# haowenz/FEM

Hardware: AMD Instinct MI355X
Metric: mapped Mreads/s (100 bp, e=3) at 1/2/4/8 MI355X + achieved HBM GB/s vs roofline (higher is better)
Workload: dtype u32/u64 integer + 32-bit Myers bit-vectors

## Files before the change

### fem_amd/csrc/fem_hip.hip

```cpp
#include "../../include/fem_hip.h"

#include <hip/hip_runtime.h>
#include <rccl/rccl.h>
#include <sched.h>
#if defined(__x86_64__)
#include <immintrin.h>
#endif

#include <algorithm>
#include <cctype>
#include <cstdio>
#include <cstdlib>
#include <cstring>
#include <condition_variable>
#include <functional>
#include <memory>
#include <atomic>
#include <chrono>
#include <mutex>
#include <string>
#include <thread>
#include <utility>
#include <vector>

#include "fem_buf.hip.h"
#include "fem_index_build.hip.h"
#include "fem_pack.h"
#include "fem_kernels.hip.h"
#include "fem_verify.hip.h"
#include "fem_seed_fast.hip.h"
#include "fem_seed_join.hip.h"
#include "fem_tail.hip.h"
#include "fem_bgzf.hip.h"

namespace {

using femb::Buf;
using femb::Event;
using femb::PinBuf;
using femb::Stream;
template <typename T>
using StageBuf = femb::Buf<T, femb::Mem::Device, femb::Grow::Half>;
template <typename T>
using PinStageBuf = femb::Buf<T, femb::Mem::Pinned, femb::Grow::Half>;

#ifndef FEM_SLOTS
#define FEM_SLOTS 4
#endif
constexpr int kSlots = FEM_SLOTS;
constexpr uint32_t kMaxReadLen = 1024;
constexpr size_t kFrontPad = 16;
constexpr size_t kPackedFrontPad = 256;
constexpr uint32_t kXcapSmall = 512, kFcap = 128, kCcap = 128;

constexpr int kTimedKernels = 16;
struct TimedLaunch {
  int kernel;
  hipEvent_t start, stop;
  bool counts = true;
};
constexpr int kMaxParts = 4;

struct Slot {
  Stream stream;
  StageBuf<uint8_t> d_bases_alloc;
  uint8_t *bases() const { return d_bases_alloc + 16; }
  StageBuf<uint64_t> d_off;
  uint64_t n_reads = 0;
  uint64_t n_bases = 0;
  uint32_t max_len = 0;
  bool staged = false;
  PinStageBuf<char> h_bases;
  PinStageBuf<uint64_t> h_off;
  uint64_t acq_reads = 0, acq_bases = 0;
  PinStageBuf<char> h_quals, h_names;
  PinStageBuf<uint64_t> h_name_off;
  StageBuf<uint8_t> d_quals, d_names;
  StageBuf<uint64_t> d_name_off;
  bool text_staged = false;
  bool host_quals = false;
  const uint64_t *qual_at = nullptr;
  Stream text_stream;
  Stream out_stream;
  Event ev_text_staged;
  Event ev_text_order;
  bool have_text_order = false;
  StageBuf<uint8_t> d_packed_alloc;
  uint8_t *packed() const { return d_packed_alloc + kPackedFrontPad; }
  StageBuf<uint32_t> d_exc_bits;
  uint32_t packed_bpr = 0;
  bool prefetch_results = false, staged_by_copy = false;
  uint64_t prefetched_reads2 = 0, prefetched_cand = 0, last_n_cand = 0;
  uint64_t h2d_bytes = 0;
  bool sent_packed = false;
  int parts = 1;
  uint32_t part_begin[kMaxParts + 1] = {0, 0, 0, 0, 0};
  Event ev_part[kMaxParts], ev_sel[kMaxParts];
  Event ev_zeroed;
  Event ev_results, ev_home;
  Buf<uint64_t> d_cand;
  Buf<uint32_t> d_meta;
  Buf<uint8_t> d_ed;
  Buf<int16_t> d_end;
  uint32_t cand_cap = 0;
  Buf<uint32_t> d_begin, d_count, d_nmap;
  Buf<uint8_t> d_ctl;
  PinBuf<uint8_t> h_ctl;
  Buf<uint64_t> d_arena;
  uint64_t arena_cap = 0;
  Buf<uint32_t> d_slow;
  uint32_t slow_cap = 0;
  StageBuf<uint2> d_sel, d_sel_hdr;
  PinBuf<uint32_t> h_begin, h_count;
  PinBuf<uint64_t> h_cand;
  PinBuf<uint8_t> h_ed;
  PinBuf<int16_t> h_end;
  StageBuf<uint8_t> d_count8;
  StageBuf<uint32_t> d_seg;
  Buf<uint64_t> d_pcand;
  Buf<uint8_t> d_ped;
  Buf<int16_t> d_pend;
  Buf<uint2> d_big;
  PinBuf<uint8_t> h_count8, h_ped;
  PinBuf<uint32_t> h_seg;
  PinBuf<uint64_t> h_pcand;
  PinBuf<int16_t> h_pend;
  PinBuf<uint2> h_big;
  bool want_packed = false;
  bool packed_enqueued = false;
  uint64_t packed_home = 0, last_n_packed = 0;
  bool packed_per_read_home = false;
  uint32_t n_packed = 0, n_big = 0;
  fem_params params{};
  bool mapped = false, synced = false;
  uint64_t stats[5] = {0, 0, 0, 0, 0};
  uint32_t n_cand = 0;
  std::vector<TimedLaunch> pending;
  std::unique_ptr<femt::Tail> tail;
  bool paired = false;
  int32_t min_insert = 0, max_insert = 0;
  uint64_t n_proper = 0;
  bool rescue = false;
  int32_t rescue_edits = 0;
  uint64_t n_rescued = 0;
  bool mapq = false;
  bool unmapped = false;
  uint64_t n_unmapped = 0;
  int32_t report_strata = -1, report_hits = -1;
  uint64_t n_filtered = 0;
  std::vector<uint16_t> pr_flag;
  std::vector<uint32_t> pr_tid, pr_pos0, pr_cigar_off, pr_cigar, pr_md_off;
  std::vector<uint8_t> pr_nm;
  std::vector<char> pr_md;
};

constexpr size_t kCtlPackCursor = 4 * sizeof(uint32_t) + 2 * sizeof(uint64_t) + 4 * sizeof(uint64_t);
constexpr size_t kCtlBytes = kCtlPackCursor + 2 * sizeof(uint32_t);
constexpr uint32_t kBigCap = 4096;
constexpr size_t kCtlWorkCursor = 128, kCtlWorkCursor2 = 192, kCtlPartStride = 128, kCtlAlloc = 1024;
static_assert(kCtlWorkCursor2 + (kMaxParts - 1) * kCtlPartStride + 64 <= kCtlAlloc, "control block layout");
static_assert(kCtlBytes <= kCtlWorkCursor, "control block layout");

}

namespace {
class StagePool {
 public:
  ~StagePool() {
    {
      std::lock_guard<std::mutex> l(m_);
      stop_ = true;
    }
    cv_.notify_all();
    for (auto &t : threads_) t.join();
  }
  void run(unsigned n, const std::function<void(unsigned)> &work) {
    if (n <= 1) return work(0u);
    {
      std::lock_guard<std::mutex> l(m_);
      while (threads_.size() + 1 < n) {
        const unsigned id = (unsigned)threads_.size() + 1;
        threads_.emplace_back([this, id] { loop(id); });
      }
      work_ = &work, n_ = n, pending_ = n - 1, ++epoch_;
    }
    cv_.notify_all();
    work(0u);
    std::unique_lock<std::mutex> l(m_);
    done_.wait(l, [&] { return pending_ == 0; });
    work_ = nullptr;
  }

 private:
  void loop(unsigned id) {
    uint64_t seen = 0;
    for (;;) {
      const std::function<void(unsigned)> *w = nullptr;
      {
        std::unique_lock<std::mutex> l(m_);
        cv_.wait(l, [&] { return stop_ || (epoch_ != seen && id < n_); });
        if (stop_) return;
        seen = epoch_, w = work_;
      }
      (*w)(id);
      std::lock_guard<std::mutex> l(m_);
      if (--pending_ == 0) done_.notify_one();
    }
  }
  std::mutex m_;
  std::condition_variable cv_, done_;
  std::vector<std::thread> threads_;
  const std::function<void(unsigned)> *work_ = nullptr;
  unsigned n_ = 0, pending_ = 0;
  uint64_t epoch_ = 0;
  bool stop_ = false;
};
}

struct fem_dev {
  femt::TextGate text_gate;
  std::unique_ptr<femz::Bgzf> bgzf;
  Buf<uint8_t> d_zin;
  Stream z_stream;
  std::recursive_mutex mu;
  int device = 0;
  std::unique_ptr<StagePool> stage_pool;
  Buf<uint8_t> d_ref_names;
  Buf<uint32_t> d_ref_name_off;
  int n_cu = 256;
  std::string err;
  Buf<uint32_t> d_lookup;
  uint64_t n_lookup = 0;
  Buf<uint64_t> d_occ;
  uint64_t n_occ = 0;
  int32_t k = 0, step = 0;
  uint64_t fast_occ_key = ~0ull;
  int fast_occ_blocks = 0;
  Buf<uint32_t> d_summary;
  Buf<uint32_t> d_occ32, d_goff, d_blkseq;
  uint32_t list_shift = 0;
  bool no_strided = false;
  bool verify_chars = false;
  Buf<uint32_t> d_freq11;
  uint32_t n_banks = 1, bank_first[5] = {0, 0, 0, 0, 0};
  Buf<uint32_t> d_bank_lo;
  uint64_t bank_limit = 0;
  uint32_t bank_seqs = 0;
  int select_occ_blocks = 0, join_occ_blocks = 0;
  uint64_t select_occ_key = ~0ull, join_occ_key = ~0ull;
  Buf<uint8_t> d_planes;
  Buf<uint8_t> d_ref_raw;
  uint64_t ref_bytes = 0;
  Buf<uint64_t> d_seq_off;
  Buf<uint32_t> d_seq_len;
  uint32_t n_seq = 0;
  std::vector<uint64_t> seq_off;
  std::vector<uint32_t> seq_len;
  Slot slot[kSlots];
  bool timing = false;
  int verify_blocks_per_cu = 0;
  int verify_packed_blocks_per_cu = 0;
  double t_ms[kTimedKernels] = {};
  uint64_t t_n[kTimedKernels] = {};
  bool force_generic = false;
  bool force_hash = false;
  bool force_dense = false;
  bool no_dense = false;
  bool tiny_buffers = false;
  femb::EventPool event_pool;
  Event ev_kernels_done;
  bool have_kernels_done = false;
  Event ev_select_done;
  bool have_select_done = false;
  bool no_overlap = false;
  Event ev_h2d_done;
  bool have_h2d_done = false;
  Stream side_stream;
  bool no_parts = false;
  int max_parts = 2;
  bool timeline = false, have_epoch = false;
  Event ev_epoch;
};

namespace {

bool testing_switch(const char *name) {
  const char *t = getenv("FEM_TESTING");
  if (!(t && t[0] == '1')) return false;
  const char *v = getenv(name);
  return v && v[0] == '1';
}

int fail(fem_dev *h, int rc, const std::string &msg) {
  if (h) {
    std::lock_guard<std::recursive_mutex> lock(h->mu);
    h->err = msg;
  }
  return rc;
}
#define FEM_LOCK(h) std::lock_guard<std::recursive_mutex> fem_lock_(h->mu)

#define HIP_TRY(h, expr)                                                                          \
  do {                                                                                            \
    hipError_t e_ = (expr);                                                                       \
    if (e_ != hipSuccess)                                                                         \
      return fail(h, e_ == hipErrorOutOfMemory ? FEM_ERR_NOMEM : FEM_ERR_HIP,                     \
                  std::string(#expr) + ": " + hipGetErrorString(e_));                             \
  } while (0)

bool params_ok(const fem_params *p) {
  return p && p->k >= 1 && p->k <= 15 && p->step >= 1 && p->step <= 16 && p->e >= 0 && p->e <= 7 && p->a >= 0 &&
         p->a <= 2;
}

femk::SeedLayout make_layout(const fem_params &p, uint32_t max_len) {
  femk::SeedLayout l{};
  const uint32_t R = (uint32_t)(p.e + 1 + p.a);
  const uint32_t lg = (uint32_t)(p.k / p.step + (p.k % p.step ? 1 : 0));
  const uint32_t n_groups = 2u * (uint32_t)p.step;
  uint32_t smax = max_len >= (uint32_t)p.k ? max_len - (uint32_t)p.k + 1u : 1u;
  int c = (int)(smax / (uint32_t)p.step) - (int)(R * lg) + 2;
  uint32_t cmax = (uint32_t)std::max(c, 2);
  l.smax = smax;
  l.cmax = cmax;
  l.cw = (cmax + 31u) / 32u;
  l.n_words = (max_len + 15u) / 16u + 2u;
  l.xcap = kXcapSmall, l.fcap = kFcap, l.ccap = kCcap;
  uint32_t o = 0;
  auto take = [&](uint32_t bytes) {
    uint32_t at = o;
    o += (bytes + 15u) & ~15u;
    return at;
  };
  l.pkw = take(l.n_words * 4u);
  l.nkw = take(l.n_words * 4u);
  l.sf = take(2u * smax * 8u);
  l.dp_rows = take(n_groups * 2u * cmax * 4u);
  l.dp_bits = take(std::max(n_groups * R * l.cw * 4u, n_groups * R * 8u));
  l.picked = take(n_groups * R * 16u);
  l.rb = take(2u * (R + 1u) * 4u);
  l.X = take(l.xcap * 8u);
  l.F = take(l.fcap * 8u);
  l.A = take(l.ccap * 8u);
  l.B = take(l.ccap * 8u);
  l.wave_bytes = o;
  return l;
}

femk::SeedLayout make_layout_fast(const fem_params &p, uint32_t max_len, bool hash) {
  femk::SeedLayout l{};
  const uint32_t R = (uint32_t)(p.e + 1 + p.a);
  const uint32_t n_groups = 2u * (uint32_t)p.step;
  l.smax = max_len >= (uint32_t)p.k ? max_len - (uint32_t)p.k + 1u : 1u;
  l.n_words = (max_len + 15u) / 16u + 2u;
  l.xcap = 64;
  uint32_t o = 0;
  auto take = [&](uint32_t bytes) {
    uint32_t at = o;
    o += (bytes + 15u) & ~15u;
    return at;
  };
  if (hash) {
    l.pkw = take(l.n_words * 4u);
    l.nkw = take(l.n_words * 4u);
  }
  if (hash) l.sf = take(std::max(2u * l.smax * 8u, 2u * 64u * 8u));
  l.dp_bits = take(std::max(n_groups, femk::kGroupQueue) * R * 8u);
  if (hash) {
    l.X = take(64u * 8u);
    l.A = take(femk::kListScratchBytes);
  }
  l.B = take(2u * femk::kReadBlock * 8u);
  if (!hash) {
    const uint32_t blk_chars = femk::kReadBlock * std::min(max_len, 256u);
    l.strm_words = blk_chars / 16u + 3u;
    l.strm = take(3u * l.strm_words * 4u);
    const uint32_t q_at = o;
    l.F = take(femk::kQueueBytes);
    const uint32_t g0 = l.smax / (uint32_t)femk::kStep;
    const uint32_t n_used = g0 > (uint32_t)femk::kLg ? g0 - (uint32_t)femk::kLg + 1u : 1u;
    l.gq_cap = std::max(384u, n_groups * n_used);
    l.gq = take(std::max(l.gq_cap * 4u + femk::kGroupQueue * 16u + 2u * 32u * 4u, femk::kFlushScratchBytes));
    l.blk_bytes = blk_chars + 32u;
    l.blk = q_at;
    if (o < q_at + l.blk_bytes) take(q_at + l.blk_bytes - o);
  }
  if (hash) {
    l.xcap = (uint32_t)femk::bloom_chunks((int)R) * 64u;
    l.F = take(femk::bloom_slots((int)R) / 16u * 4u);
  }
  l.wave_bytes = o;
  return l;
}

femk::SeedLayout make_layout_select(const fem_params &p, uint32_t max_len) {
  femk::SeedLayout l{};
  const uint32_t R = (uint32_t)(p.e + 1 + p.a);
  l.smax = max_len >= (uint32_t)p.k ? max_len - (uint32_t)p.k + 1u : 1u;
  const uint32_t g_max = std::min<uint32_t>((l.smax + 2u) / 3u, femk::kSelMaxCols - 1u + 4u * R);
  l.gstride = 3u * g_max + 2u;
  l.gstride += l.gstride & 1u;
  if (!((l.gstride >> 1) & 1u)) l.gstride += 2u;
  l.nb = std::max<uint32_t>(1u, std::min<uint32_t>(femk::kReadBlock, 3100u / (2u * 2u * l.gstride)));
  l.strm_words = (l.nb * max_len + 15u) / 16u + 2u;
  uint32_t o = 0;
  auto take = [&](uint32_t bytes) {
    uint32_t at = o;
    o += (bytes + 15u) & ~15u;
    return at;
  };
  l.rb = take((femk::kReadBlock + 2u) * 8u);
  l.rinfo = take(4u * femk::kReadBlock * 4u);
  l.strm = take(2u * l.strm_words * 4u);
  l.fq = take(l.nb * 2u * l.gstride * 2u + 256u);
  l.wave_bytes = o;
  return l;
}

femk::SeedLayout make_layout_join(const fem_params &p, bool banked, bool padded = false) {
  femk::SeedLayout l{};
  const uint32_t R = (uint32_t)(p.e + 1 + p.a);
  uint32_t o = 0;
  auto take = [&](uint32_t bytes) {
    uint32_t at = o;
    o += (bytes + 15u) & ~15u;
    return at;
  };
  l.sf = take(2u * 64u * 4u);
  l.X = take(64u * 4u);
  l.A = take(3u * (femk::dense_flag_cap((int)R) + 1u) * 4u);
  l.B = take(2u * femk::kReadBlock * 8u);
  l.F = take(femk::join_bitmap_words((int)R, padded) * 4u);
  if (banked) l.gq = take(2u * 64u * 8u);
  l.wave_bytes = o;
  l.picked = 0;
  return l;
}

typedef void (*SeedKernel)(femk::SeedParams);
template <size_t... I>
SeedKernel select_kernel_of(int R, bool banked, std::index_sequence<I...>) {
  static const SeedKernel k[2][femk::kMaxR] = {{femk::seed_select_kernel<(int)I + 1, false>...}, {femk::seed_select_kernel<(int)I + 1, true>...}};
  return k[banked][std::min(std::max(R, 1), femk::kMaxR) - 1];
}
template <size_t... I>
SeedKernel fast_kernel_of(int R, bool hash, std::index_sequence<I...>) {
  static const SeedKernel k[2][femk::kMaxR] = {{femk::seed_fast_kernel<(int)I + 1, false>...}, {femk::seed_fast_kernel<(int)I + 1, true>...}};
  return k[hash][std::min(std::max(R, 1), femk::kMaxR) - 1];
}
SeedKernel select_kernel(int R, bool banked) { return select_kernel_of(R, banked, std::make_index_sequence<femk::kMaxR>{}); }
SeedKernel fast_kernel(int R, bool hash) { return fast_kernel_of(R, hash, std::make_index_sequence<femk::kMaxR>{}); }
SeedKernel join_kernel(int R, int which) {
  static const SeedKernel k[3][femk::kMaxR] = {
      {femk::seed_join_kernel_r1, femk::seed_join_kernel_r2, femk::seed_join_kernel_r3, femk::seed_join_kernel_r4, femk::seed_join_kernel_r5,
       femk::seed_join_kernel_r6, femk::seed_join_kernel_r7, femk::seed_join_kernel_r8, femk::seed_join_kernel_r9, femk::seed_join_kernel_r10},
      {femk::seed_join_banked_kernel_r1, femk::seed_join_banked_kernel_r2, femk::seed_join_banked_kernel_r3, femk::seed_join_banked_kernel_r4,
       femk::seed_join_banked_kernel_r5, femk::seed_join_banked_kernel_r6, femk::seed_join_banked_kernel_r7, femk::seed_join_banked_kernel_r8,
       femk::seed_join_banked_kernel_r9, femk::seed_join_banked_kernel_r10},
      {femk::seed_join_kernel_padded_r1, femk::seed_join_kernel_padded_r2, femk::seed_join_kernel_padded_r3, femk::seed_join_kernel_padded_r4,
       femk::seed_join_kernel_padded_r5, femk::seed_join_kernel_padded_r6, femk::seed_join_kernel_padded_r7, femk::seed_join_kernel_padded_r8,
       femk::seed_join_kernel_padded_r9, femk::seed_join_kernel_padded_r10}};
  return k[which][std::min(std::max(R, 1), femk::kMaxR) - 1];
}

int blocks_per_cu(const void *kernel, int block, uint32_t lds) {
  int nb = 0;
  return hipOccupancyMaxActiveBlocksPerMultiprocessor(&nb, kernel, block, lds) == hipSuccess ? nb : 0;
}
uint32_t kernel_regs(int R, bool join, int which = 0) {
  static std::atomic<uint32_t> cache[3][2][femk::kMaxR + 1] = {};
  std::atomic<uint32_t> &slot = cache[which][join ? 1 : 0][std::min(std::max(R, 1), femk::kMaxR)];
  uint32_t c = slot.load(std::memory_order_relaxed);
  if (c) return c;
  hipFuncAttributes a{};
  const void *f = join ? (const void *)join_kernel(R, which) : (const void *)select_kernel(R, which == 1);
  c = hipFuncGetAttributes(&a, f) == hipSuccess && a.numRegs > 0 ? (uint32_t)a.numRegs : 128u;
  slot.store(c, std::memory_order_relaxed);
  return c;
}
void launch_select(int R, bool banked, dim3 grid, dim3 block, uint32_t lds, hipStream_t st, const femk::SeedParams &sp) {
  hipLaunchKernelGGL(select_kernel(R, banked), grid, block, lds, st, sp);
}
void launch_join(int R, int which, dim3 grid, dim3 block, uint32_t lds, hipStream_t st, const femk::SeedParams &sp) {
  hipLaunchKernelGGL(join_kernel(R, which), grid, block, lds, st, sp);
}
void launch_fast(int R, bool hash, dim3 grid, dim3 block, uint32_t lds, hipStream_t st, const femk::SeedParams &sp) {
  hipLaunchKernelGGL(fast_kernel(R, hash), grid, block, lds, st, sp);
}

struct Span {
  fem_dev *h;
  Slot &s;
  hipStream_t st;
  TimedLaunch t;
  bool on;
  Span(fem_dev *h_, Slot &s_, int id, hipStream_t st_) : h(h_), s(s_), st(st_), t{id, nullptr, nullptr, false}, on(h_->timing && h_->timeline) {
    if (on) {
      t.start = h->event_pool.get(), t.stop = h->event_pool.get();
      (void)hipEventRecord(t.start, st);
    }
  }
  ~Span() {
    if (on) {
      (void)hipEventRecord(t.stop, st);
      s.pending.push_back(t);
    }
  }
};

void drain_timing(fem_dev *h, Slot &s) {
  for (auto &t : s.pending) {
    float ms = 0.f;
    if (hipEventElapsedTime(&ms, t.start, t.stop) == hipSuccess && t.kernel < kTimedKernels) {
      h->t_ms[t.kernel] += ms;
      h->t_n[t.kernel] += t.counts ? 1 : 0;
    }
    if (h->timeline && h->have_epoch) {
      float a = 0.f, b = 0.f;
      if (hipEventElapsedTime(&a, h->ev_epoch, t.start) == hipSuccess && hipEventElapsedTime(&b, h->ev_epoch, t.stop) == hipSuccess)
        fprintf(stderr, "TL slot %d id %2d  %9.3f %9.3f  (%.3f)\n", (int)(&s - h->slot), t.kernel, a, b, b - a);
    }
    h->event_pool.put(t.start);
    h->event_pool.put(t.stop);
  }
  s.pending.clear();
}

int ensure_outputs(fem_dev *h, Slot &s) {
  if ((size_t)s.n_reads > s.d_nmap.size() || !s.d_nmap) {
    const size_t cap = std::max<size_t>((size_t)s.n_reads, 1);
    s.d_nmap.release();
    HIP_TRY(h, femb::alloc_all(cap * 2, s.d_begin, s.d_count));
    HIP_TRY(h, s.d_nmap.ensure(cap));
  }
  if (!s.d_cand || s.cand_cap == 0) {
    uint64_t want = 2 * s.n_reads + (5u << 20);
    if (h->tiny_buffers) want = 512;
    want = std::min<uint64_t>(want, 0xFFFFFFF0ull);
    s.cand_cap = 0;
    HIP_TRY(h, femb::alloc_all(want, s.d_cand, s.d_meta, s.d_ed, s.d_end));
    s.cand_cap = (uint32_t)want;
  }
  HIP_TRY(h, s.d_ctl.ensure(kCtlAlloc));
  HIP_TRY(h, s.h_ctl.ensure(kCtlBytes));
  if (!s.d_arena) {
    s.arena_cap = h->tiny_buffers ? 256u : (4u << 20);
    HIP_TRY(h, s.d_arena.ensure(s.arena_cap));
  }
  {
    const double avg_bucket = (double)h->n_occ / (double)(h->n_lookup ? h->n_lookup : 1);
    uint64_t want = avg_bucket > 1.0 ? s.n_reads + (1u << 20) : (1u << 18);
    if (h->tiny_buffers) want = s.d_slow ? s.slow_cap : 32;
    if (want > s.slow_cap || !s.d_slow) {
      s.d_slow.release();
      HIP_TRY(h, s.d_slow.ensure(want));
      s.slow_cap = (uint32_t)want;
    }
  }
  return FEM_OK;
}

int grow_candidates(fem_dev *h, Slot &s, uint64_t want) {
  if (want > 0xFFFFFFF0ull) return fail(h, FEM_ERR_UNSUPPORTED, "more than 2^32 candidates in one batch; split the batch");
  s.cand_cap = 0;
// ... 4 lines not shown

int h2d_begin(fem_dev *h, Slot &s) {
  if (h->have_h2d_done) HIP_TRY(h, hipStreamWaitEvent(s.stream, h->ev_h2d_done, 0));
  return FEM_OK;
}
int h2d_end(fem_dev *h, Slot &s) {
  HIP_TRY(h, hipEventRecord(h->ev_h2d_done, s.stream));
  h->have_h2d_done = true;
  return FEM_OK;
}
bool device_idle(fem_dev *h) {
  return (!h->have_kernels_done || hipEventQuery(h->ev_kernels_done) == hipSuccess) &&
         (!h->have_select_done || hipEventQuery(h->ev_select_done) == hipSuccess);
}
constexpr uint64_t kPartMinReads = 1u << 16;

hipStream_t d2h_begin(fem_dev *h, Slot &s) {
  (void)h;
  return s.stream;
}
int d2h_end(fem_dev *h, Slot &s, hipStream_t st) {
  if (st == s.stream) return FEM_OK;
  HIP_TRY(h, hipEventRecord(s.ev_home, st));
  HIP_TRY(h, hipStreamWaitEvent(s.stream, s.ev_home, 0));
  return FEM_OK;
}

template <typename Launch>
int timed_launch(fem_dev *h, Slot &s, int id, hipStream_t st, bool counts, Launch &&launch) {
  TimedLaunch t{id, nullptr, nullptr, counts};
  if (h->timing) {
    t.start = h->event_pool.get(), t.stop = h->event_pool.get();
    HIP_TRY(h, hipEventRecord(t.start, st));
  }
  launch();
  HIP_TRY(h, hipGetLastError());
  if (h->timing) {
    HIP_TRY(h, hipEventRecord(t.stop, st));
    s.pending.push_back(t);
  }
  return FEM_OK;
}

int enqueue_pack(fem_dev *h, Slot &s, bool kernel, bool send_home) {
  const size_t n2 = (size_t)s.n_reads * 2, n_seg = (n2 + 255) / 256;
  int rc;
  HIP_TRY(h, s.d_count8.ensure(n2 + 16));
  HIP_TRY(h, s.d_seg.ensure(n_seg + 4));
  if (s.d_pcand.size() < s.cand_cap || !s.d_pcand) HIP_TRY(h, femb::alloc_all(s.cand_cap, s.d_pcand, s.d_ped, s.d_pend));
  HIP_TRY(h, s.d_big.ensure(kBigCap));
  HIP_TRY(h, s.h_count8.ensure(n2 + 16));
  HIP_TRY(h, s.h_seg.ensure(n_seg + 4));
  HIP_TRY(h, s.h_big.ensure(kBigCap));
  if (kernel) {
    femk::PackParams pp{};
    pp.cand_begin = s.d_begin, pp.cand_count = s.d_count, pp.cand = s.d_cand, pp.ed = s.d_ed, pp.end = s.d_end;
    pp.ctr = (const uint32_t *)s.d_ctl.get(), pp.n_strands = (uint32_t)n2;
    pp.count8 = s.d_count8, pp.seg_begin = s.d_seg, pp.pcand = s.d_pcand, pp.ped = s.d_ped, pp.pend = s.d_pend, pp.pcap = (uint32_t)s.d_pcand.size();
    pp.cursor = (uint32_t *)(s.d_ctl + kCtlPackCursor), pp.big = s.d_big, pp.big_cap = kBigCap;
    const uint32_t grid = (uint32_t)std::max<size_t>(1, (n_seg + femk::kPackSegs - 1) / femk::kPackSegs);
    if ((rc = timed_launch(h, s, 6, s.stream, true, [&] { hipLaunchKernelGGL(femk::pack_results_kernel, dim3(grid), dim3(256), 0, s.stream, pp); }))) return rc;
    s.packed_enqueued = true;
  }
  if (send_home) {
    hipStream_t st = d2h_begin(h, s);
    {
      Span span(h, s, 21, st);
      HIP_TRY(h, hipMemcpyAsync(s.h_count8, s.d_count8, n2, hipMemcpyDeviceToHost, st));
      HIP_TRY(h, hipMemcpyAsync(s.h_seg, s.d_seg, n_seg * sizeof(uint32_t), hipMemcpyDeviceToHost, st));
      s.packed_per_read_home = true;
      const size_t guess = std::min<size_t>({(size_t)(s.last_n_packed + s.last_n_packed / 32 + 1024), s.h_pcand.size(), s.d_pcand.size()});
      if (s.last_n_packed && s.h_pcand && guess) {
        HIP_TRY(h, hipMemcpyAsync(s.h_pcand, s.d_pcand, guess * sizeof(uint64_t), hipMemcpyDeviceToHost, st));
        HIP_TRY(h, hipMemcpyAsync(s.h_ped, s.d_ped, guess * sizeof(uint8_t), hipMemcpyDeviceToHost, st));
        HIP_TRY(h, hipMemcpyAsync(s.h_pend, s.d_pend, guess * sizeof(int16_t), hipMemcpyDeviceToHost, st));
        s.packed_home = guess;
      }
    }
    if ((rc = d2h_end(h, s, st))) return rc;
  }
  return FEM_OK;
}

int launch_batch(fem_dev *h, Slot &s) {
  const fem_params &p = s.params;
  uint32_t *d_ctr = (uint32_t *)s.d_ctl.get();
  unsigned long long *d_arena_ctr = (unsigned long long *)(s.d_ctl + 4 * sizeof(uint32_t));
  unsigned long long *d_stats = (unsigned long long *)(s.d_ctl + 4 * sizeof(uint32_t) + 2 * sizeof(uint64_t));
  int parts = 1;
  uint32_t part_begin[kMaxParts + 1] = {0, 0, 0, 0, 0};
  const bool copied_in_parts = s.parts > 1;
  {
    const int R_ = p.e + 1 + p.a;
    const bool dense_overlap = !h->force_generic && p.k == femk::kK && p.step == femk::kStep && R_ >= 1 && R_ <= femk::kMaxR && h->d_occ32 &&
                               h->d_freq11 && !h->no_overlap;
    if (dense_overlap && !h->no_parts && s.n_reads >= 2 * kPartMinReads && (copied_in_parts || device_idle(h))) {
      parts = copied_in_parts ? s.parts : (int)std::min<uint64_t>((uint64_t)h->max_parts, s.n_reads / kPartMinReads);
      for (int q = 0; q <= parts; ++q)
        part_begin[q] = copied_in_parts ? s.part_begin[q] : q == parts ? (uint32_t)s.n_reads : (uint32_t)((s.n_reads * q / parts) & ~63ull);
    }
    s.parts = 1;
  }
  if (parts > 1) {
    if (h->have_select_done) HIP_TRY(h, hipStreamWaitEvent(h->side_stream, h->ev_select_done, 0));
    HIP_TRY(h, hipMemsetAsync(s.d_ctl, 0, kCtlAlloc, h->side_stream));
  } else {
    HIP_TRY(h, hipMemsetAsync(s.d_ctl, 0, kCtlAlloc, s.stream));
  }

  femk::SeedParams sp{};
  sp.bases = s.bases();
  sp.read_off = s.d_off;
  sp.n_reads = (uint32_t)s.n_reads;
  sp.read_begin = 0;
  sp.lookup = h->d_lookup;
  sp.occ = h->d_occ;
  sp.inf32 = (uint32_t)h->n_occ;
  sp.seq_len = h->d_seq_len;
  sp.e = p.e, sp.a = p.a, sp.R = p.e + 1 + p.a, sp.k = p.k, sp.step = p.step;
  sp.lg = p.k / p.step + (p.k % p.step ? 1 : 0);
  sp.cand = s.d_cand, sp.cand_meta = s.d_meta, sp.cand_cap = s.cand_cap;
  sp.cand_begin = s.d_begin, sp.cand_count = s.d_count;
  sp.ctr = d_ctr;
  sp.work_cursor = (uint32_t *)(s.d_ctl + kCtlWorkCursor);
  sp.stats = d_stats;
  sp.arena = s.d_arena, sp.arena_cap = s.arena_cap, sp.arena_ctr = d_arena_ctr;
  sp.lay = make_layout(p, std::max<uint32_t>(s.max_len, (uint32_t)p.k));

  sp.n_seq = h->n_seq;
  sp.summary = h->d_summary;
  sp.slow_queue = s.d_slow, sp.slow_cap = s.slow_cap;
  sp.work_queue = nullptr;
  const int R = p.e + 1 + p.a;
  const bool use_fast = !h->force_generic && p.k == femk::kK && p.step == femk::kStep && R >= 1 && R <= femk::kMaxR;

  auto shape = [&](const femk::SeedLayout &lay, uint32_t *wpb_out, uint32_t *lds_out, uint32_t *grid_out) {
    uint32_t wpb = std::min<uint32_t>(4u, std::max<uint32_t>(1u, (64u * 1024u) / lay.wave_bytes));
    uint32_t lds_bytes = wpb * lay.wave_bytes;
    uint32_t waves_per_cu = std::min<uint32_t>(32u, (160u * 1024u / lds_bytes) * wpb);
    uint64_t blocks_wanted = (s.n_reads + wpb - 1) / wpb;
    uint64_t blocks_resident = (uint64_t)h->n_cu * std::max<uint32_t>(1u, waves_per_cu / wpb);
    *wpb_out = wpb, *lds_out = lds_bytes;
    *grid_out = (uint32_t)std::max<uint64_t>(1, std::min<uint64_t>(blocks_wanted, blocks_resident * 4));
  };
  if (sp.lay.wave_bytes > 64u * 1024u) return fail(h, FEM_ERR_UNSUPPORTED, "read too long for the device path");

  if (s.n_reads) {
    int rc;
    const bool split_dense = use_fast && h->d_occ32 && h->d_freq11;
    const bool overlap = split_dense && !h->no_overlap;
    if (!overlap && h->have_kernels_done) HIP_TRY(h, hipStreamWaitEvent(s.stream, h->ev_kernels_done, 0));
    femk::VerifyParams vp{};
    vp.bases = s.bases(), vp.read_off = s.d_off;
    vp.planes = h->d_planes, vp.seq_off = h->d_seq_off;
    vp.cand = s.d_cand, vp.cand_meta = s.d_meta;
    vp.ctr = d_ctr, vp.cand_cap = s.cand_cap, vp.e = p.e;
    vp.ed = s.d_ed, vp.end = s.d_end;
    vp.n_map = s.d_nmap, vp.stats = d_stats;
    HIP_TRY(h, hipMemsetAsync(s.d_nmap, 0, (size_t)s.n_reads * sizeof(uint32_t), s.stream));
    const bool verify_packed = s.sent_packed && !h->verify_chars;
    if (verify_packed) vp.packed = s.packed(), vp.exc_bits = s.d_exc_bits, vp.bpr = s.packed_bpr, vp.len = s.max_len;
    void (*const verify)(femk::VerifyParams) = verify_packed ? femk::verify_kernel_packed : femk::verify_kernel;
    int &v_per_cu = verify_packed ? h->verify_packed_blocks_per_cu : h->verify_blocks_per_cu;
    if (v_per_cu == 0) {
      const int nb = blocks_per_cu((const void *)verify, 256, 0);
      v_per_cu = nb > 0 ? nb : 4;
    }
    const uint32_t vgrid = (uint32_t)h->n_cu * (uint32_t)v_per_cu;
    if (split_dense) {
      const uint32_t max_len = std::max<uint32_t>(s.max_len, (uint32_t)p.k);
      const bool banked = h->n_banks > 1;
      const size_t want_sel = (size_t)s.n_reads * 6u * (size_t)R * h->n_banks;
      HIP_TRY(h, s.d_sel.ensure(want_sel));
      HIP_TRY(h, s.d_sel_hdr.ensure((size_t)s.n_reads));
      femk::SeedParams fp = sp;
      fp.occ32 = h->d_occ32, fp.list_shift = h->list_shift, fp.goff = h->d_goff, fp.blkseq = h->d_blkseq;
      fp.freq11 = h->d_freq11, fp.sel = s.d_sel, fp.sel_hdr = s.d_sel_hdr;
      fp.n_banks = h->n_banks, fp.bank_lo = h->d_bank_lo, fp.n_buckets = (uint32_t)(h->n_lookup - 1);
      fp.blk_stride = (femk::kDenseRemap >> femk::kDenseBlkShift) + 1u;
      for (uint32_t b = 0; b <= femk::kDenseMaxBanks; ++b) fp.bank_first[b] = h->bank_first[b];
      uint32_t select_lds = 0, select_threads = 256;
      fp.lay = make_layout_select(p, max_len);
      if (fp.lay.wave_bytes > 64u * 1024u) return fail(h, FEM_ERR_UNSUPPORTED, "read too long for the device path");
      const femk::SeedLayout lay_select = fp.lay;
      femk::SeedLayout lay_join = make_layout_join(p, banked, !banked && h->list_shift != 0);
      const uint32_t wpb_s = std::min<uint32_t>(4u, std::max<uint32_t>(1u, (64u * 1024u) / lay_select.wave_bytes));
      const uint32_t wpb_j = std::min<uint32_t>(4u, std::max<uint32_t>(1u, (60u * 1024u) / lay_join.wave_bytes));
      lay_join.picked = wpb_j * lay_join.wave_bytes;
      const uint32_t lds_j = wpb_j * lay_join.wave_bytes + 64u * 8u;
      const int which = banked ? 1 : h->list_shift ? 2 : 0;
      uint64_t per_cu_s, per_cu_j;
      {
        const uint32_t lds_bytes = wpb_s * lay_select.wave_bytes;
        const uint64_t key = ((uint64_t)banked << 48) | ((uint64_t)R << 40) | lds_bytes;
        if (h->select_occ_key != key) h->select_occ_key = key, h->select_occ_blocks = blocks_per_cu((const void *)select_kernel(R, banked), (int)(64u * wpb_s), lds_bytes);
        per_cu_s = h->select_occ_blocks > 0 ? (uint64_t)h->select_occ_blocks : std::max<uint64_t>(1, 160u * 1024u / lds_bytes);
        if (overlap) per_cu_s = 1;
        select_lds = lds_bytes, select_threads = 64u * wpb_s;
      }
      {
        const uint64_t key = ((uint64_t)which << 48) | ((uint64_t)R << 40) | lds_j;
        if (h->join_occ_key != key) h->join_occ_key = key, h->join_occ_blocks = blocks_per_cu((const void *)join_kernel(R, which), (int)(64u * wpb_j), lds_j);
        per_cu_j = h->join_occ_blocks > 0 ? (uint64_t)h->join_occ_blocks : std::max<uint64_t>(1, 160u * 1024u / lds_j);
        if (overlap) {
          const uint32_t vj = (kernel_regs(R, true, which) + 7u) & ~7u, vs = (kernel_regs(R, false, banked ? 1 : 0) + 7u) & ~7u;
          const uint32_t wj = 64u * wpb_j / 256u ? 64u * wpb_j / 256u : 1u, ws = select_threads / 256u ? select_threads / 256u : 1u;
          const uint32_t lj = (lds_j + 511u) & ~511u, ls = (select_lds + 511u) & ~511u;
          while (per_cu_j > 1 && (per_cu_j * wj * vj + ws * vs > 512u || per_cu_j * lj + ls > 160u * 1024u || per_cu_j * wj + ws > 8u)) --per_cu_j;
        }
      }
      if (parts > 1 && !copied_in_parts) {
        HIP_TRY(h, hipEventRecord(s.ev_zeroed, s.stream));
        HIP_TRY(h, hipStreamWaitEvent(h->side_stream, s.ev_zeroed, 0));
      }
      for (int q = 0; q < parts; ++q) {
        const uint32_t r_lo = parts > 1 ? part_begin[q] : 0u, r_hi = parts > 1 ? part_begin[q + 1] : (uint32_t)s.n_reads;
        const uint64_t blocks_of_reads = ((uint64_t)(r_hi - r_lo) + femk::kReadBlock - 1) / femk::kReadBlock;
        fp.read_begin = r_lo, fp.n_reads = r_hi;
        hipStream_t st_sel = parts > 1 ? h->side_stream : s.stream;
        {
          fp.lay = lay_select;
          if (parts > 1) {
            if (copied_in_parts) HIP_TRY(h, hipStreamWaitEvent(st_sel, s.ev_part[q], 0));
          } else if (overlap && h->have_select_done) {
            HIP_TRY(h, hipStreamWaitEvent(s.stream, h->ev_select_done, 0));
          }
          const uint32_t grid = (uint32_t)std::max<uint64_t>(1, std::min<uint64_t>((blocks_of_reads + wpb_s - 1) / wpb_s, (uint64_t)h->n_cu * per_cu_s));
          fp.work_cursor = (uint32_t *)(s.d_ctl + kCtlWorkCursor + (size_t)q * kCtlPartStride);
          rc = timed_launch(h, s, 8, st_sel, q == 0, [&] { launch_select(R, banked, dim3(grid), dim3(64u * wpb_s), select_lds, st_sel, fp); });
          if (rc) return rc;
          if (parts > 1) {
            HIP_TRY(h, hipEventRecord(s.ev_sel[q], st_sel));
            HIP_TRY(h, hipStreamWaitEvent(s.stream, s.ev_sel[q], 0));
          }
          if (overlap && q + 1 == parts) {
            HIP_TRY(h, hipEventRecord(h->ev_select_done, st_sel));
            h->have_select_done = true;
          }
          if (overlap && q == 0 && h->have_kernels_done) HIP_TRY(h, hipStreamWaitEvent(s.stream, h->ev_kernels_done, 0));
        }
        {
          fp.lay = lay_join;
          const uint32_t grid = (uint32_t)std::max<uint64_t>(1, std::min<uint64_t>((blocks_of_reads + wpb_j - 1) / wpb_j, (uint64_t)h->n_cu * per_cu_j));
          fp.work_cursor = (uint32_t *)(s.d_ctl + kCtlWorkCursor2 + (size_t)q * kCtlPartStride);
          rc = timed_launch(h, s, 0, s.stream, q == 0, [&] { launch_join(R, which, dim3(grid), dim3(64u * wpb_j), lds_j, s.stream, fp); });
          if (rc) return rc;
        }
      }
      sp.work_queue = s.d_slow;
    } else if (use_fast) {
      femk::SeedParams fp = sp;
      const bool hash = h->force_hash || (double)h->n_occ > (double)h->n_lookup;
      fp.lay = make_layout_fast(p, std::max<uint32_t>(s.max_len, (uint32_t)p.k), hash);
      uint32_t wpb, lds_bytes, grid;
      shape(fp.lay, &wpb, &lds_bytes, &grid);
      {
        const uint64_t key = ((uint64_t)R << 40) | ((uint64_t)hash << 32) | lds_bytes;
        if (h->fast_occ_key != key) h->fast_occ_key = key, h->fast_occ_blocks = blocks_per_cu((const void *)fast_kernel((int)R, hash), (int)(64u * wpb), lds_bytes);
        static const uint64_t mult = testing_switch("FEM_TESTING") && getenv("FEM_GRID_MULT") ? (uint64_t)std::max(1, atoi(getenv("FEM_GRID_MULT"))) : 1;
        const uint64_t per_cu = h->fast_occ_blocks > 0 ? (uint64_t)h->fast_occ_blocks : std::max<uint64_t>(1, 160u * 1024u / lds_bytes);
        const uint64_t wanted = (s.n_reads + (uint64_t)femk::kReadBlock * wpb - 1) / ((uint64_t)femk::kReadBlock * wpb);
        grid = (uint32_t)std::max<uint64_t>(1, std::min<uint64_t>(wanted, (uint64_t)h->n_cu * per_cu * mult));
      }
      auto launch_range = [&](uint32_t lo, uint32_t hi) {
        femk::SeedParams q = fp;
        q.read_begin = lo, q.n_reads = hi;
        dim3 g(grid), b(64u * wpb);
        launch_fast((int)R, hash, g, b, lds_bytes, s.stream, q);
      };
      rc = timed_launch(h, s, 0, s.stream, true, [&] { launch_range(0, (uint32_t)s.n_reads); });
      if (rc) return rc;
      sp.work_queue = s.d_slow;
    }
    {
      uint32_t wpb, lds_bytes, grid;
      shape(sp.lay, &wpb, &lds_bytes, &grid);
      rc = timed_launch(h, s, 2, s.stream, true, [&] { hipLaunchKernelGGL(femk::seed_filter_kernel, dim3(grid), dim3(64u * wpb), lds_bytes, s.stream, sp); });
      if (rc) return rc;
    }
    rc = timed_launch(h, s, 1, s.stream, true, [&] { hipLaunchKernelGGL(verify, dim3(vgrid), dim3(256), 0, s.stream, vp); });
    if (rc) return rc;
    s.packed_enqueued = false, s.packed_home = 0, s.packed_per_read_home = false;
    if (s.want_packed && split_dense && (rc = enqueue_pack(h, s, true, false))) return rc;
    HIP_TRY(h, hipEventRecord(h->ev_kernels_done, s.stream));
    h->have_kernels_done = true;
    if (s.want_packed && (rc = enqueue_pack(h, s, !split_dense, true))) return rc;
  } else {
    s.packed_enqueued = false, s.packed_home = 0, s.packed_per_read_home = false;
// ... 88 lines not shown
    (void)hipGetLastError();
    return FEM_OK;
  };
  uint32_t list_shift = 0;
  const bool strided_pays = h->force_dense || h->n_occ >= (n_buckets << 4);
  if (n_banks == 1 && !h->no_strided && strided_pays) {
    const size_t words = ((size_t)n_buckets + femk::kDensePadBuckets) << femk::kDenseListShift;
    bool ok = h->d_occ32.ensure(words) == hipSuccess;
    if (ok) {
      hipLaunchKernelGGL(femk::dense_pad_kernel, dim3((uint32_t)h->n_cu * 16u), dim3(256), 0, 0, (uint4 *)h->d_occ32.get(), (uint64_t)(words / 4));
      ok = hipGetLastError() == hipSuccess;
    }
    if (ok) {
      list_shift = femk::kDenseListShift;
    } else {
      h->d_occ32.release();
      (void)hipGetLastError();
    }
  }
  if (h->d_goff.ensure(goff.size()) != hipSuccess || h->d_blkseq.ensure(blkseq.size()) != hipSuccess ||
      (!list_shift && h->d_occ32.ensure(h->n_occ + 256) != hipSuccess) || h->d_freq11.ensure((size_t)femk::kX11 * 4u) != hipSuccess ||
      (n_banks > 1 && h->d_bank_lo.ensure((size_t)(n_banks - 1) * n_buckets) != hipSuccess) || d_bad.ensure(1) != hipSuccess)
    return decline();
  if (hipMemset(d_bad, 0, sizeof(uint32_t)) != hipSuccess ||
      hipMemcpy(h->d_goff, goff.data(), goff.size() * sizeof(uint32_t), hipMemcpyHostToDevice) != hipSuccess ||
      hipMemcpy(h->d_blkseq, blkseq.data(), blkseq.size() * sizeof(uint32_t), hipMemcpyHostToDevice) != hipSuccess) {
    (void)decline();
    return fail(h, FEM_ERR_HIP, "dense tables: copy to the device failed");
  }
  femk::BankFirst bf{};
  bf.n = n_banks;
  for (uint32_t b = 0; b <= femk::kDenseMaxBanks; ++b) bf.first[b] = bank_first[b];
  if (list_shift)
    hipLaunchKernelGGL(femk::dense_occ32_strided_kernel, dim3((uint32_t)h->n_cu * 8u), dim3(256), 0, 0, h->d_occ, h->d_lookup, (uint32_t)n_buckets, h->d_goff,
                       h->n_seq, h->d_occ32, d_bad);
  else
    hipLaunchKernelGGL(femk::dense_occ32_kernel, dim3((uint32_t)h->n_cu * 8u), dim3(256), 0, 0, h->d_occ, h->n_occ, h->d_goff, h->n_seq, bf,
                       h->d_occ32, d_bad);
  uint32_t bad = 0;
  if (hipGetLastError() != hipSuccess || hipMemcpy(&bad, d_bad, sizeof bad, hipMemcpyDeviceToHost) != hipSuccess) {
    (void)decline();
    return fail(h, FEM_ERR_HIP, "dense tables: building the 32-bit occurrence table failed");
  }
  if (bad) return decline();
  d_bad.release();
  for (uint32_t b = 1; b < n_banks; ++b)
    hipLaunchKernelGGL(femk::bank_split_kernel, dim3((uint32_t)h->n_cu * 8u), dim3(256), 0, 0, h->d_occ, h->d_lookup, (uint32_t)n_buckets, bank_first[b],
                       h->d_bank_lo + (size_t)(b - 1) * n_buckets);
  h->n_banks = n_banks, h->list_shift = list_shift;
  for (uint32_t b = 0; b <= femk::kDenseMaxBanks; ++b) h->bank_first[b] = bank_first[b];
  hipLaunchKernelGGL(femk::freq11_kernel, dim3((uint32_t)h->n_cu * 8u), dim3(256), 0, 0, h->d_lookup, h->d_freq11);
  HIP_TRY(h, hipGetLastError());
  HIP_TRY(h, hipDeviceSynchronize());
  return FEM_OK;
}

struct CommSet {
  std::vector<int> devs;
  std::vector<ncclComm_t> comms;
  std::vector<Buf<uint64_t>> bufs;
};
std::mutex g_comm_mu;
CommSet *g_comm = nullptr;
void destroy_comm_set() {
  if (!g_comm) return;
  for (size_t i = 0; i < g_comm->devs.size(); ++i) {
    (void)hipSetDevice(g_comm->devs[i]);
    g_comm->bufs[i].release();
    if (g_comm->comms[i]) ncclCommDestroy(g_comm->comms[i]);
  }
  delete g_comm;
  g_comm = nullptr;
}

int check_slot(fem_dev *h, int slot) {
  if (!h) return FEM_ERR_INVALID;
  if (slot < 0 || slot >= kSlots) return fail(h, FEM_ERR_INVALID, "slot out of range");
  return FEM_OK;
}


using fempack::pack_bases;

int enqueue_packed(fem_dev *h, Slot &s, uint64_t n, uint32_t len, uint64_t n_exc) {
  const uint32_t bpr = fempack::bytes_per_read(len);
  const uint64_t code_bytes = fempack::code_bytes(n, len), n_bases = n * (uint64_t)len;
  const uint64_t total = code_bytes + n_exc * 5u;
  int rc;
  HIP_TRY(h, s.d_packed_alloc.ensure(kPackedFrontPad + (size_t)total + 64));
  HIP_TRY(h, s.d_bases_alloc.ensure(kFrontPad + (size_t)n_bases + 64));
  HIP_TRY(h, s.d_off.ensure((size_t)n + 1));
  HIP_TRY(h, s.d_exc_bits.ensure((size_t)n / 32 + 2));
  s.parts = 1;
  if (!h->no_parts && !h->no_overlap && n_exc == 0 && n >= 2 * kPartMinReads && device_idle(h))
    s.parts = (int)std::min<uint64_t>((uint64_t)h->max_parts, n / kPartMinReads);
  for (int q = 0; q <= s.parts; ++q) s.part_begin[q] = q == s.parts ? (uint32_t)n : (uint32_t)((n * q / s.parts) & ~63ull);
  HIP_TRY(h, hipMemsetAsync(s.d_exc_bits, 0, ((size_t)n / 32 + 1) * sizeof(uint32_t), s.stream));
  hipLaunchKernelGGL(femk::uniform_offsets_kernel, dim3((uint32_t)std::min<uint64_t>((n + 256) / 256, (uint64_t)h->n_cu * 8u)), dim3(256), 0,
                     s.stream, s.d_off, n, len);
  if ((rc = h2d_begin(h, s))) return rc;
  for (int q = 0; q < s.parts; ++q) {
    const uint64_t r0 = s.part_begin[q], r1 = s.part_begin[q + 1];
    const uint64_t b0 = r0 * bpr, b1 = q + 1 == s.parts ? total : r1 * bpr;
    Span span(h, s, 20, s.stream);
    if (b1 > b0) HIP_TRY(h, hipMemcpyAsync(s.packed() + b0, s.h_bases + b0, b1 - b0, hipMemcpyHostToDevice, s.stream));
    if (q + 1 == s.parts && (rc = h2d_end(h, s))) return rc;
    if (r1 > r0) {
      const uint32_t grid = (uint32_t)std::min<uint64_t>(((r1 - r0) * bpr + 255) / 256, (uint64_t)h->n_cu * 16u);
      hipLaunchKernelGGL(femk::unpack_reads_kernel, dim3(grid), dim3(256), 0, s.stream, (const uint8_t *)s.packed() + b0, r1 - r0, len, bpr,
                         s.bases() + r0 * len);
    }
    if (s.parts > 1) HIP_TRY(h, hipEventRecord(s.ev_part[q], s.stream));
  }
  if (n_exc) {
    const dim3 g((uint32_t)std::min<uint64_t>((n_exc + 255) / 256, (uint64_t)h->n_cu * 4u));
    hipLaunchKernelGGL(femk::scatter_chars_kernel, g, dim3(256), 0, s.stream, (const uint32_t *)(s.packed() + code_bytes),
                       (const uint8_t *)(s.packed() + code_bytes + 4u * n_exc), n_exc, s.bases());
    hipLaunchKernelGGL(femk::mark_exception_reads_kernel, g, dim3(256), 0, s.stream, (const uint32_t *)(s.packed() + code_bytes), n_exc, len,
                       s.d_exc_bits);
  }
  s.packed_bpr = bpr;
  HIP_TRY(h, hipGetLastError());
  s.n_reads = n, s.n_bases = n_bases, s.max_len = len;
  s.staged = true, s.mapped = false, s.synced = false;
  s.h2d_bytes = total, s.sent_packed = true;
  return FEM_OK;
}

unsigned stage_threads(uint64_t n_reads) {
  unsigned want = 12;
  if (const char *e = getenv("FEM_STAGE_THREADS")) want = (unsigned)std::max(1, atoi(e));
  const unsigned hw = std::thread::hardware_concurrency();
  return (unsigned)std::max<uint64_t>(1, std::min<uint64_t>({(uint64_t)(hw ? hw : 1), (uint64_t)want, n_reads / 65536 + 1}));
}

}

extern "C" {

const char *fem_strerror(int rc) {
  switch (rc) {
    case FEM_OK: return "ok";
    case FEM_ERR_INVALID: return "invalid argument";
    case FEM_ERR_HIP: return "HIP runtime error";
    case FEM_ERR_NOMEM: return "out of memory";
    case FEM_ERR_STATE: return "call order violated";
    case FEM_ERR_UNSUPPORTED: return "input not supported by the device path";
    case FEM_ERR_RCCL: return "RCCL error";
    default: return "unknown error";
  }
}

const char *fem_dev_last_error(const fem_dev *h) { return h ? h->err.c_str() : "null handle"; }

static std::atomic<int> g_blocking_waits{0};
int fem_set_blocking_waits(int on) {
  g_blocking_waits.store(on ? 1 : 0);
  return FEM_OK;
}

int fem_dev_open(int device, fem_dev **out) {
  if (!out) return FEM_ERR_INVALID;
  *out = nullptr;
  int n = 0;
  if (hipGetDeviceCount(&n) != hipSuccess || n <= 0) return FEM_ERR_HIP;
  if (device < 0 || device >= n) return FEM_ERR_INVALID;
  fem_dev *h = new (std::nothrow) fem_dev();
  if (!h) return FEM_ERR_NOMEM;
  h->device = device;
  if (hipSetDevice(device) != hipSuccess) {
    delete h;
    return FEM_ERR_HIP;
  }
  if (g_blocking_waits.load() || testing_switch("FEM_BLOCKING_SYNC")) (void)hipSetDeviceFlags(hipDeviceScheduleBlockingSync);
  hipDeviceProp_t prop;
  if (hipGetDeviceProperties(&prop, device) == hipSuccess) h->n_cu = prop.multiProcessorCount;
  for (int i = 0; i < kSlots; ++i) {
    if (h->slot[i].stream.create(hipStreamNonBlocking) != hipSuccess) {
      delete h;
      return FEM_ERR_HIP;
    }
  }
  bool ok_ev = h->ev_kernels_done.create(hipEventDisableTiming) == hipSuccess && h->ev_select_done.create(hipEventDisableTiming) == hipSuccess &&
               h->ev_h2d_done.create(hipEventDisableTiming) == hipSuccess && h->side_stream.create(hipStreamNonBlocking) == hipSuccess;
  for (int i = 0; ok_ev && i < kSlots; ++i) {
    Slot &sl = h->slot[i];
    ok_ev = sl.ev_zeroed.create(hipEventDisableTiming) == hipSuccess && sl.ev_results.create(hipEventDisableTiming) == hipSuccess &&
            sl.ev_home.create(hipEventDisableTiming) == hipSuccess;
    for (int q = 0; ok_ev && q < kMaxParts; ++q)
      ok_ev = sl.ev_part[q].create(hipEventDisableTiming) == hipSuccess && sl.ev_sel[q].create(hipEventDisableTiming) == hipSuccess;
  }
  if (!ok_ev) {
    (void)fem_dev_close(h);
    return FEM_ERR_HIP;
  }
  if (testing_switch("FEM_TESTING")) {
    h->no_overlap = testing_switch("FEM_NO_OVERLAP");
    h->no_parts = testing_switch("FEM_NO_PARTS");
    if (const char *mp = getenv("FEM_PARTS")) h->max_parts = std::min(kMaxParts, std::max(1, atoi(mp)));
    h->timeline = testing_switch("FEM_TIMELINE");
    if (h->timeline && h->ev_epoch.create() == hipSuccess && hipEventRecord(h->ev_epoch, h->side_stream) == hipSuccess)
      h->timing = true, h->have_epoch = true;
    h->force_generic = testing_switch("FEM_FORCE_GENERIC");
    h->force_hash = testing_switch("FEM_FORCE_HASH");
    h->force_dense = testing_switch("FEM_FORCE_DENSE");
    h->no_dense = testing_switch("FEM_NO_DENSE");
    h->no_strided = testing_switch("FEM_NO_STRIDED");
    h->verify_chars = testing_switch("FEM_VERIFY_CHARS");
    h->tiny_buffers = testing_switch("FEM_TEST_TINY_BUFFERS");
    if (const char *bl = getenv("FEM_TEST_BANK_BASES")) h->bank_limit = strtoull(bl, nullptr, 10);
    if (const char *bs = getenv("FEM_TEST_BANK_SEQS")) h->bank_seqs = (uint32_t)strtoul(bs, nullptr, 10);
  }
  *out = h;
  return FEM_OK;
}

int fem_dev_close(fem_dev *h) {
  if (!h) return FEM_ERR_INVALID;
  {
    std::lock_guard<std::mutex> lock(g_comm_mu);
    if (g_comm && std::find(g_comm->devs.begin(), g_comm->devs.end(), h->device) != g_comm->devs.end()) destroy_comm_set();
  }
  (void)hipSetDevice(h->device);
  (void)hipDeviceSynchronize();
  for (auto &s : h->slot) drain_timing(h, s);
  delete h;
  return FEM_OK;
}

int fem_dev_limits(const fem_dev *h, uint32_t *max_read_len, int32_t *n_slots) {
  if (!h) return FEM_ERR_INVALID;
  if (max_read_len) *max_read_len = kMaxReadLen;
  if (n_slots) *n_slots = kSlots;
  return FEM_OK;
}

int fem_dev_upload_index(fem_dev *h, int32_t k, int32_t step, const uint32_t *lookup, uint64_t n_lookup,
                         const uint64_t *occ, uint64_t n_occ) {
  if (!h || !lookup || (!occ && n_occ)) return FEM_ERR_INVALID;
  if (k < 1 || k > 15 || step < 1) return fail(h, FEM_ERR_INVALID, "k must be 1..15 and step >= 1");
  if (n_lookup != (1ull << (2 * k)) + 1) return fail(h, FEM_ERR_INVALID, "lookup table must have 4^k + 1 entries");
  if (n_occ > 0xFFFFFFFFull) return fail(h, FEM_ERR_INVALID, "occurrence table larger than its uint32 prefix sums");
  HIP_TRY(h, hipSetDevice(h->device));
  h->d_lookup.release(), h->d_occ.release();
  HIP_TRY(h, h->d_lookup.ensure(n_lookup));
  HIP_TRY(h, h->d_occ.ensure(std::max<uint64_t>(n_occ, 1)));
  HIP_TRY(h, hipMemcpy(h->d_lookup, lookup, n_lookup * sizeof(uint32_t), hipMemcpyHostToDevice));
  if (n_occ) HIP_TRY(h, hipMemcpy(h->d_occ, occ, n_occ * sizeof(uint64_t), hipMemcpyHostToDevice));
  h->n_lookup = n_lookup, h->n_occ = n_occ, h->k = k, h->step = step;
  int rc = refresh_summary(h);
  return rc ? rc : refresh_dense(h);
}

namespace {
int make_codes(fem_dev *h, Buf<uint8_t> *codes) {
  const uint64_t total = h->ref_bytes;
  HIP_TRY(h, codes->ensure(total + 128));
  HIP_TRY(h, hipMemcpy(*codes, h->d_ref_raw, total, hipMemcpyDeviceToDevice));
  HIP_TRY(h, hipMemset(*codes + total, 4, 128));
  if (total) {
    hipLaunchKernelGGL(femk::ref_encode_kernel, dim3((uint32_t)h->n_cu * 8u), dim3(256), 0, 0, codes->get(), total);
    HIP_TRY(h, hipGetLastError());
    HIP_TRY(h, hipDeviceSynchronize());
  }
  return FEM_OK;
}
}

int fem_dev_upload_reference(fem_dev *h, uint32_t n_seq, const char *const *seq, const uint32_t *seq_len) {
  if (!h || !seq || !seq_len || n_seq == 0) return FEM_ERR_INVALID;
  HIP_TRY(h, hipSetDevice(h->device));
  h->seq_off.assign(n_seq, 0);
  h->seq_len.assign(seq_len, seq_len + n_seq);
  uint64_t total = 0;
  for (uint32_t i = 0; i < n_seq; ++i) {
    h->seq_off[i] = total;
    total += seq_len[i];
  }
  auto drop_reference = [&]() {
    h->d_ref_raw.release(), h->d_seq_off.release(), h->d_seq_len.release(), h->d_planes.release();
    h->ref_bytes = 0, h->n_seq = 0;
  };
  drop_reference();
  HIP_TRY(h, h->d_ref_raw.ensure(total + 128));
  HIP_TRY(h, h->d_seq_off.ensure(n_seq));
  HIP_TRY(h, h->d_seq_len.ensure(n_seq));
  for (uint32_t i = 0; i < n_seq; ++i)
    if (seq_len[i]) HIP_TRY(h, hipMemcpy(h->d_ref_raw + h->seq_off[i], seq[i], seq_len[i], hipMemcpyHostToDevice));
  HIP_TRY(h, hipMemset(h->d_ref_raw + total, 0, 128));
  HIP_TRY(h, hipMemcpy(h->d_seq_off, h->seq_off.data(), n_seq * sizeof(uint64_t), hipMemcpyHostToDevice));
  HIP_TRY(h, hipMemcpy(h->d_seq_len, h->seq_len.data(), n_seq * sizeof(uint32_t), hipMemcpyHostToDevice));
// ... 20 lines not shown
  return refresh_dense(h);
}

int fem_dev_build_index(fem_dev *h, int32_t k, int32_t step, uint32_t *lookup_out, uint64_t *occ_out, uint64_t occ_cap,
                        uint64_t *n_occ_out) {
  if (!h) return FEM_ERR_INVALID;
  if (!h->d_ref_raw) return fail(h, FEM_ERR_STATE, "upload the reference before building the index");
  if (k < 1 || k > 15 || step < 1) return fail(h, FEM_ERR_INVALID, "k must be 1..15 and step >= 1");
  HIP_TRY(h, hipSetDevice(h->device));
  h->d_lookup.release(), h->d_occ.release();
  uint64_t n_occ = 0;
  std::string err;
  Buf<uint8_t> codes;
  int rc = make_codes(h, &codes);
  if (rc) return rc;
  rc = femix::build_index(codes, h->seq_off, h->seq_len, k, step, h->n_cu, &h->d_lookup, &h->d_occ, &n_occ, &err);
  codes.release();
  if (rc != FEM_OK) return fail(h, rc, err);
  h->n_lookup = (1ull << (2 * k)) + 1, h->n_occ = n_occ, h->k = k, h->step = step;
  if ((rc = refresh_summary(h))) return rc;
  if ((rc = refresh_dense(h))) return rc;
  if (n_occ_out) *n_occ_out = n_occ;
  if (lookup_out)
    HIP_TRY(h, hipMemcpy(lookup_out, h->d_lookup, h->n_lookup * sizeof(uint32_t), hipMemcpyDeviceToHost));
  if (occ_out) {
    if (occ_cap < n_occ) return fail(h, FEM_ERR_INVALID, "occ_out too small");
    if (n_occ) HIP_TRY(h, hipMemcpy(occ_out, h->d_occ, n_occ * sizeof(uint64_t), hipMemcpyDeviceToHost));
  }
  return FEM_OK;
}

int fem_dev_fetch_index(fem_dev *h, uint32_t *lookup_out, uint64_t *occ_out, uint64_t occ_cap) {
  if (!h) return FEM_ERR_INVALID;
  if (!h->d_lookup) return fail(h, FEM_ERR_STATE, "no index is resident");
  HIP_TRY(h, hipSetDevice(h->device));
  if (lookup_out) HIP_TRY(h, hipMemcpy(lookup_out, h->d_lookup, h->n_lookup * sizeof(uint32_t), hipMemcpyDeviceToHost));
  if (occ_out) {
    if (occ_cap < h->n_occ) return fail(h, FEM_ERR_INVALID, "occ_out too small");
    if (h->n_occ) HIP_TRY(h, hipMemcpy(occ_out, h->d_occ, h->n_occ * sizeof(uint64_t), hipMemcpyDeviceToHost));
  }
  return FEM_OK;
}

int fem_dev_acquire_stage(fem_dev *h, int slot, uint64_t n_reads_cap, uint64_t n_bases_cap, char **bases, uint64_t **offsets) {
  int rc = check_slot(h, slot);
  if (rc) return rc;
  FEM_LOCK(h);
  if (!bases || !offsets) return fail(h, FEM_ERR_INVALID, "null output pointer");
  if (n_reads_cap > 0x3FFFFFF0ull) return fail(h, FEM_ERR_UNSUPPORTED, "more than 2^30 reads in one batch");
  Slot &s = h->slot[slot];
  HIP_TRY(h, hipSetDevice(h->device));
  HIP_TRY(h, hipStreamSynchronize(s.stream));
  if (s.out_stream) HIP_TRY(h, hipStreamSynchronize(s.out_stream));
  drain_timing(h, s);
  HIP_TRY(h, s.h_bases.ensure((size_t)n_bases_cap + 64));
  HIP_TRY(h, s.h_off.ensure((size_t)n_reads_cap + 1));
  s.staged = false, s.mapped = false, s.synced = false, s.text_staged = false;
  s.acq_reads = n_reads_cap, s.acq_bases = n_bases_cap;
  *bases = s.h_bases, *offsets = s.h_off;
  return FEM_OK;
}

int fem_dev_commit_stage(fem_dev *h, int slot, uint64_t n_reads, uint32_t max_len) {
  int rc = check_slot(h, slot);
  if (rc) return rc;
  FEM_LOCK(h);
  Slot &s = h->slot[slot];
  if (!s.h_bases || !s.h_off) return fail(h, FEM_ERR_STATE, "acquire the slot's staging buffers first");
  if (n_reads > s.acq_reads) return fail(h, FEM_ERR_INVALID, "more reads than the staging buffers were acquired for");
  if (max_len > kMaxReadLen)
    return fail(h, FEM_ERR_UNSUPPORTED, "read longer than the device path supports (" + std::to_string(kMaxReadLen) + ")");
  const uint64_t n_bases = n_reads ? s.h_off[n_reads] : 0;
  if (n_reads && (s.h_off[0] != 0 || n_bases > s.acq_bases)) return fail(h, FEM_ERR_INVALID, "staged offsets must start at 0 and end inside the buffer");
  HIP_TRY(h, hipSetDevice(h->device));
  HIP_TRY(h, s.d_bases_alloc.ensure(kFrontPad + (size_t)n_bases + 64));
  HIP_TRY(h, s.d_off.ensure((size_t)n_reads + 1));
  if ((rc = h2d_begin(h, s))) return rc;
  if (n_bases) HIP_TRY(h, hipMemcpyAsync(s.bases(), s.h_bases, n_bases, hipMemcpyHostToDevice, s.stream));
  if (n_reads) HIP_TRY(h, hipMemcpyAsync(s.d_off, s.h_off, (n_reads + 1) * sizeof(uint64_t), hipMemcpyHostToDevice, s.stream));
  if ((rc = h2d_end(h, s))) return rc;
  s.parts = 1;
  s.n_reads = n_reads, s.n_bases = n_bases, s.max_len = max_len;
  s.staged = true, s.mapped = false, s.synced = false;
  s.h2d_bytes = n_bases + (n_reads ? (n_reads + 1) * sizeof(uint64_t) : 0), s.sent_packed = false, s.staged_by_copy = false;
  return FEM_OK;
}

int fem_dev_commit_stage_uniform(fem_dev *h, int slot, uint64_t n_reads, uint32_t read_len) {
  int rc = check_slot(h, slot);
  if (rc) return rc;
  FEM_LOCK(h);
  Slot &s = h->slot[slot];
  if (!s.h_bases) return fail(h, FEM_ERR_STATE, "acquire the slot's staging buffers first");
  if (read_len > kMaxReadLen)
    return fail(h, FEM_ERR_UNSUPPORTED, "read longer than the device path supports (" + std::to_string(kMaxReadLen) + ")");
  const uint64_t n_bases = n_reads * (uint64_t)read_len;
  if (n_reads > s.acq_reads || n_bases > s.acq_bases) return fail(h, FEM_ERR_INVALID, "more reads than the staging buffers were acquired for");
  HIP_TRY(h, hipSetDevice(h->device));
  HIP_TRY(h, s.d_bases_alloc.ensure(kFrontPad + (size_t)n_bases + 64));
  HIP_TRY(h, s.d_off.ensure((size_t)n_reads + 1));
  if ((rc = h2d_begin(h, s))) return rc;
  if (n_bases) HIP_TRY(h, hipMemcpyAsync(s.bases(), s.h_bases, n_bases, hipMemcpyHostToDevice, s.stream));
  if ((rc = h2d_end(h, s))) return rc;
  s.parts = 1;
  hipLaunchKernelGGL(femk::uniform_offsets_kernel, dim3((uint32_t)std::min<uint64_t>((n_reads + 256) / 256, (uint64_t)h->n_cu * 8u)), dim3(256), 0,
                     s.stream, s.d_off, n_reads, read_len);
  HIP_TRY(h, hipGetLastError());
  s.n_reads = n_reads, s.n_bases = n_bases, s.max_len = read_len;
  s.staged = true, s.mapped = false, s.synced = false;
  s.h2d_bytes = n_bases, s.sent_packed = false, s.staged_by_copy = false;
  return FEM_OK;
}

int fem_dev_packed_layout(uint64_t n_reads, uint32_t read_len, uint32_t *bytes_per_read, uint64_t *exc_offset, uint64_t *exc_cap) {
  if (read_len == 0 || read_len > kMaxReadLen) return FEM_ERR_INVALID;
  const uint64_t n_bases = n_reads * (uint64_t)read_len, cb = fempack::code_bytes(n_reads, read_len);
  if (bytes_per_read) *bytes_per_read = fempack::bytes_per_read(read_len);
  if (exc_offset) *exc_offset = cb;
  if (exc_cap) *exc_cap = std::min<uint64_t>((n_bases + 64 - std::min<uint64_t>(cb, n_bases + 64)) / 5u, n_bases / 16u);
  return FEM_OK;
}

int fem_dev_commit_stage_packed(fem_dev *h, int slot, uint64_t n_reads, uint32_t read_len, uint64_t n_exceptions) {
  int rc = check_slot(h, slot);
  if (rc) return rc;
  FEM_LOCK(h);
  Slot &s = h->slot[slot];
  if (!s.h_bases) return fail(h, FEM_ERR_STATE, "acquire the slot's staging buffers first");
  if (read_len == 0 && n_reads) return fail(h, FEM_ERR_INVALID, "packed batches hold reads of one non-zero length");
  if (read_len > kMaxReadLen)
    return fail(h, FEM_ERR_UNSUPPORTED, "read longer than the device path supports (" + std::to_string(kMaxReadLen) + ")");
  const uint64_t n_bases = n_reads * (uint64_t)read_len;
  if (n_reads > s.acq_reads || n_bases > s.acq_bases) return fail(h, FEM_ERR_INVALID, "more reads than the staging buffers were acquired for");
  if (n_bases >= 0xFFFFFFF0ull) return fail(h, FEM_ERR_UNSUPPORTED, "a packed batch holds fewer than 2^32 bases; split the batch");
  const uint64_t code_bytes = fempack::code_bytes(n_reads, read_len);
  if (code_bytes + n_exceptions * 5u > s.acq_bases + 64 || n_exceptions > n_bases / 16u)
    return fail(h, FEM_ERR_INVALID, "more exceptions than a packed batch may carry (fem_dev_packed_layout): commit the characters instead");
  const uint32_t *pos = (const uint32_t *)(s.h_bases + code_bytes);
  for (uint64_t i = 0; i < n_exceptions; ++i)
    if (pos[i] >= n_bases) return fail(h, FEM_ERR_INVALID, "exception position outside the batch");
  HIP_TRY(h, hipSetDevice(h->device));
  if ((rc = enqueue_packed(h, s, n_reads, read_len, n_exceptions))) return rc;
  s.staged_by_copy = true;
  return FEM_OK;
}

int fem_dev_stage_reads(fem_dev *h, int slot, const fem_read_batch *reads) {
  int rc = check_slot(h, slot);
  if (rc) return rc;
  if (!reads || (reads->n_reads && (!reads->bases || !reads->offsets))) return fail(h, FEM_ERR_INVALID, "null read batch");
  if (reads->n_reads > 0x3FFFFFF0ull) return fail(h, FEM_ERR_UNSUPPORTED, "more than 2^30 reads in one batch");
  const uint64_t n = reads->n_reads;
  const uint64_t base0 = n ? reads->offsets[0] : 0;
  if (n && reads->offsets[n] < base0) return fail(h, FEM_ERR_INVALID, "read offsets must be ascending");
  const uint64_t n_bases = n ? reads->offsets[n] - base0 : 0;
  char *hb = nullptr;
  uint64_t *ho = nullptr;
  if ((rc = fem_dev_acquire_stage(h, slot, n, n_bases, &hb, &ho))) return rc;
  Slot &s = h->slot[slot];
  const unsigned n_thr = stage_threads(n);
  if (!h->stage_pool) h->stage_pool.reset(new (std::nothrow) StagePool());
  if (!h->stage_pool) return fail(h, FEM_ERR_NOMEM, "out of host memory");
  auto run_threads = [&](unsigned nt, const std::function<void(unsigned)> &work) { h->stage_pool->run(nt, work); };
  std::vector<uint32_t> t_max(n_thr, 0), t_min(n_thr, 0xFFFFFFFFu);
  std::atomic<int> bad{0};
  run_threads(n_thr, [&](unsigned t) {
    const uint64_t r_lo = n * t / n_thr, r_hi = n * (t + 1) / n_thr;
    uint32_t mx = 0, mn = 0xFFFFFFFFu;
    for (uint64_t i = r_lo; i < r_hi; ++i) {
      const uint64_t o0 = reads->offsets[i], o1 = reads->offsets[i + 1];
      if (o1 < o0) {
        bad.store(1);
        return;
      }
      const uint64_t len = o1 - o0;
      if (len > kMaxReadLen) {
        bad.store(2);
        return;
      }
      mx = std::max<uint32_t>(mx, (uint32_t)len), mn = std::min<uint32_t>(mn, (uint32_t)len);
    }
    t_max[t] = mx, t_min[t] = mn;
  });
  if (bad.load() == 1) return fail(h, FEM_ERR_INVALID, "read offsets must be ascending");
  if (bad.load() == 2)
    return fail(h, FEM_ERR_UNSUPPORTED, "read longer than the device path supports (" + std::to_string(kMaxReadLen) + ")");
  uint32_t max_len = 0, min_len = 0xFFFFFFFFu;
  for (unsigned t = 0; t < n_thr; ++t) max_len = std::max(max_len, t_max[t]), min_len = std::min(min_len, t_min[t]);
  const bool no_pack = testing_switch("FEM_NO_PACK");
  if (n && min_len == max_len && max_len > 0 && n_bases < 0xFFFFFFF0ull && !no_pack) {
    const uint32_t len = max_len, bpr = (len + 3u) / 4u;
    const uint64_t code_bytes = (n * bpr + 7u) & ~7ull;
    const uint64_t exc_cap = (n_bases + 64 - std::min<uint64_t>(code_bytes, n_bases + 64)) / 5u;
    std::vector<std::vector<uint64_t>> exc(n_thr);
    const uint8_t *src = (const uint8_t *)reads->bases + base0;
    constexpr uint64_t kPiece = 32768;
    std::atomic<uint64_t> next_piece{0};
    run_threads(n_thr, [&](unsigned t) {
      for (;;) {
        const uint64_t r_lo = next_piece.fetch_add(1, std::memory_order_relaxed) * kPiece;
        if (r_lo >= n) break;
        const uint64_t r_hi = std::min(n, r_lo + kPiece);
        if ((len & 3u) == 0u) {
          pack_bases(src + r_lo * len, (r_hi - r_lo) * len, (uint8_t *)hb + r_lo * bpr, r_lo * len, exc[t]);
        } else {
          for (uint64_t i = r_lo; i < r_hi; ++i) pack_bases(src + i * len, len, (uint8_t *)hb + i * bpr, i * len, exc[t]);
        }
      }
    });
    uint64_t n_exc = 0;
    for (const auto &v : exc) n_exc += v.size();
    if (n_exc <= exc_cap && n_exc <= n_bases / 16u) {
      uint32_t *he = (uint32_t *)(hb + code_bytes);
      uint8_t *hc = (uint8_t *)(he + n_exc);
      for (const auto &v : exc)
        for (uint64_t x : v) *he++ = (uint32_t)(x >> 8), *hc++ = (uint8_t)x;
      {
        FEM_LOCK(h);
        if ((rc = enqueue_packed(h, s, n, len, n_exc))) return rc;
      }
      s.staged_by_copy = true;
      return FEM_OK;
    }
  }
  run_threads(n_thr, [&](unsigned t) {
    const uint64_t r_lo = n * t / n_thr, r_hi = n * (t + 1) / n_thr;
    for (uint64_t i = r_lo; i < r_hi; ++i) ho[i] = reads->offsets[i] - base0;
    if (r_hi == n) ho[n] = reads->offsets[n] - base0;
    if (r_hi > r_lo) memcpy(hb + (reads->offsets[r_lo] - base0), reads->bases + reads->offsets[r_lo], reads->offsets[r_hi] - reads->offsets[r_lo]);
  });
  if (n == 0) ho[0] = 0;
  rc = fem_dev_commit_stage(h, slot, n, max_len);
  s.staged_by_copy = true;
  return rc;
}

int fem_dev_stage_info(fem_dev *h, int slot, uint64_t *h2d_bytes, int32_t *packed) {
  int rc = check_slot(h, slot);
  if (rc) return rc;
  if (h2d_bytes) *h2d_bytes = h->slot[slot].h2d_bytes;
  if (packed) *packed = h->slot[slot].sent_packed ? 1 : 0;
  return FEM_OK;
}

int fem_dev_map_staged(fem_dev *h, int slot, const fem_params *p) {
  int rc = check_slot(h, slot);
  if (rc) return rc;
  FEM_LOCK(h);
  if (!params_ok(p)) return fail(h, FEM_ERR_INVALID, "parameters out of range (k 1..15, step 1..16, e 0..7, a 0..2)");
  if (!h->d_lookup || !h->d_ref_raw || !h->d_planes) return fail(h, FEM_ERR_STATE, "index and reference must be uploaded first");
  if (p->k != h->k) return fail(h, FEM_ERR_INVALID, "k differs from the uploaded index");
  Slot &s = h->slot[slot];
  if (!s.staged) return fail(h, FEM_ERR_STATE, "no reads staged in this slot");
  HIP_TRY(h, hipSetDevice(h->device));
  s.params = *p;
  if ((rc = ensure_outputs(h, s))) return rc;
  return launch_batch(h, s);
}

int fem_dev_sync(fem_dev *h, int slot) {
  int rc = check_slot(h, slot);
  if (rc) return rc;
  Slot &s = h->slot[slot];
  if (!s.mapped) return fail(h, FEM_ERR_STATE, "nothing was mapped in this slot");
  HIP_TRY(h, hipSetDevice(h->device));
  if (s.synced) return FEM_OK;
  for (int attempt = 0; attempt < 8; ++attempt) {
    HIP_TRY(h, hipStreamSynchronize(s.stream));
    FEM_LOCK(h);
    drain_timing(h, s);
    const uint32_t *ctr = (const uint32_t *)s.h_ctl.get();
    const uint64_t *arena_ctr = (const uint64_t *)(s.h_ctl + 4 * sizeof(uint32_t));
    const uint64_t *st = (const uint64_t *)(s.h_ctl + 4 * sizeof(uint32_t) + 2 * sizeof(uint64_t));
    uint32_t flags = ctr[1];
    if (flags & femk::kFlagTooLarge)
      return fail(h, FEM_ERR_UNSUPPORTED, "a read selects more than 2^31 occurrence entries in one seed group");
    if (flags == 0) {
      s.n_cand = ctr[0];
      s.n_packed = ((const uint32_t *)(s.h_ctl + kCtlPackCursor))[0], s.n_big = ((const uint32_t *)(s.h_ctl + kCtlPackCursor))[1];
      s.stats[0] = s.n_reads;
      s.stats[1] = st[3];
      s.stats[2] = st[0];
      s.stats[3] = st[1];
      s.stats[4] = st[2];
      s.synced = true;
      return FEM_OK;
    }
    if (flags & femk::kFlagCandOverflow) {
      uint64_t want = (uint64_t)ctr[0] + ctr[0] / 8 + 1024;
      if ((rc = grow_candidates(h, s, std::min<uint64_t>(want, 0xFFFFFFF0ull)))) return rc;
    }
    if (flags & femk::kFlagQueueOverflow) {
      uint64_t want = (uint64_t)ctr[2] + ctr[2] / 8 + 4096;
      s.d_slow.release();
      s.slow_cap = 0;
      if (s.d_slow.ensure(want) != hipSuccess) return fail(h, FEM_ERR_NOMEM, "slow-read queue does not fit in device memory");
      s.slow_cap = (uint32_t)std::min<uint64_t>(want, 0xFFFFFFF0ull);
    }
    if (flags & femk::kFlagArenaOverflow) {
      uint64_t want = arena_ctr[1] + arena_ctr[1] / 8 + 1024;
      s.d_arena.release();
      if (s.d_arena.ensure(want) != hipSuccess) {
        s.arena_cap = 0;
        return fail(h, FEM_ERR_NOMEM, "scratch arena for oversized seed lists does not fit in device memory; use smaller batches");
      }
      s.arena_cap = want;
    }
    if ((rc = launch_batch(h, s))) return rc;
  }
  return fail(h, FEM_ERR_HIP, "batch kept overflowing its scratch buffers");
}

int fem_dev_fetch_stats(fem_dev *h, int slot, uint64_t stats[5]) {
  int rc = fem_dev_sync(h, slot);
  if (rc) return rc;
  if (stats) memcpy(stats, h->slot[slot].stats, sizeof(uint64_t) * 5);
  h->slot[slot].prefetch_results = false;
  return FEM_OK;
}

int fem_dev_fetch(fem_dev *h, int slot, fem_batch_result *out) {
  int rc = fem_dev_sync(h, slot);
  if (rc) return rc;
  if (!out) return fail(h, FEM_ERR_INVALID, "null result");
  Slot &s = h->slot[slot];
  const size_t n2 = (size_t)s.n_reads * 2, nc = s.n_cand;
  bool regrown = false;
// ... 208 lines not shown
  if (s.have_text_order) HIP_TRY(h, hipStreamWaitEvent(s.text_stream, s.ev_text_order, 0));
  if (with_quals && s.n_bases) HIP_TRY(h, hipMemcpyAsync(s.d_quals, s.h_quals, s.n_bases, hipMemcpyHostToDevice, s.text_stream));
  if (n_name_bytes) HIP_TRY(h, hipMemcpyAsync(s.d_names, s.h_names, n_name_bytes, hipMemcpyHostToDevice, s.text_stream));
  HIP_TRY(h, hipMemcpyAsync(s.d_name_off, s.h_name_off, (n_reads + 1) * sizeof(uint64_t), hipMemcpyHostToDevice, s.text_stream));
  HIP_TRY(h, hipEventRecord(s.ev_text_staged, s.text_stream));
  s.text_staged = true, s.host_quals = !with_quals, s.qual_at = nullptr;
  return FEM_OK;
}

int fem_dev_commit_text_stage(fem_dev *h, int slot, uint64_t n_reads, uint64_t n_name_bytes) { return commit_text(h, slot, n_reads, n_name_bytes, true); }
int fem_dev_commit_names_stage(fem_dev *h, int slot, uint64_t n_reads, uint64_t n_name_bytes) { return commit_text(h, slot, n_reads, n_name_bytes, false); }

int fem_dev_sam_quals(fem_dev *h, int slot, const uint64_t **qual_at, uint64_t *n_reads) {
  int rc = check_slot(h, slot);
  if (rc) return rc;
  FEM_LOCK(h);
  Slot &s = h->slot[slot];
  if (!qual_at) return fail(h, FEM_ERR_INVALID, "null output pointer");
  if (!s.host_quals || !s.qual_at) return fail(h, FEM_ERR_STATE, "the slot's last SAM text was rendered with its qualities (or there is none)");
  *qual_at = s.qual_at;
  if (n_reads) *n_reads = s.n_reads;
  return FEM_OK;
}

static int fetch_sam(fem_dev *h, int slot, fem_batch_sam *out, bool wait);
int fem_dev_fetch_sam(fem_dev *h, int slot, fem_batch_sam *out) { return fetch_sam(h, slot, out, true); }
int fem_dev_fetch_sam_nowait(fem_dev *h, int slot, fem_batch_sam *out) { return fetch_sam(h, slot, out, false); }
int fem_dev_sam_wait(fem_dev *h, int slot) {
  if (!h || slot < 0 || slot >= kSlots) return FEM_ERR_INVALID;
  Slot &s = h->slot[slot];
  if (!s.tail) return FEM_ERR_STATE;
  if (hipSetDevice(h->device) != hipSuccess) return FEM_ERR_HIP;
  return s.tail->wait_text();
}

static int rescue_input(fem_dev *h, const Slot &s, femt::RescueInput *ri) {
  if (!s.rescue) return FEM_OK;
  if ((int64_t)s.max_insert - s.min_insert > 65536)
    return fail(h, FEM_ERR_UNSUPPORTED, "mate rescue searches insert windows of at most 65536 (max_insert - min_insert)");
  ri->max_edits = s.rescue_edits;
  ri->bases = s.bases(), ri->read_off = s.d_off, ri->max_len = s.max_len;
  ri->ref_raw = h->d_ref_raw, ri->ref_bytes = h->ref_bytes + 64, ri->seq_off = h->d_seq_off, ri->seq_len = h->d_seq_len;
  return FEM_OK;
}

static femt::TailInput tail_input(const fem_dev *h, const Slot &s) {
  femt::TailInput in{};
  in.bases = s.bases(), in.read_off = s.d_off, in.n_reads = (uint32_t)s.n_reads, in.max_len = s.max_len;
  in.ref_raw = h->d_ref_raw, in.ref_bytes = h->ref_bytes + 64, in.seq_off = h->d_seq_off;
  in.planes = h->d_planes;
  if (s.sent_packed) in.packed = s.packed(), in.packed_bpr = s.packed_bpr, in.exc_bits = s.d_exc_bits;
  in.cand = s.d_cand, in.ed = s.d_ed, in.end = s.d_end, in.cand_begin = s.d_begin, in.cand_count = s.d_count;
  in.n_map = s.d_nmap, in.e = s.params.e, in.n_records = s.stats[4];
  return in;
}

struct TailFront {
  femt::TailInput in;
  femt::TailOutput t;
  hipStream_t stream;
  double ms[3], ms_sync, ms_run;
  std::chrono::steady_clock::time_point t_in;
};

static int tail_records(fem_dev *h, int slot, const void *out, bool copy_records, bool device_quals, TailFront *f) {
  f->t_in = std::chrono::steady_clock::now();
  auto since = [&]() { return std::chrono::duration<double, std::milli>(std::chrono::steady_clock::now() - f->t_in).count(); };
  int rc = fem_dev_sync(h, slot);
  if (rc) return rc;
  f->ms_sync = since();
  if (!out) return fail(h, FEM_ERR_INVALID, "null result");
  Slot &s = h->slot[slot];
  const bool text = !copy_records, paired = text && s.paired;
  if (text && !s.text_staged) return fail(h, FEM_ERR_STATE, "qualities and names of this batch were not committed (fem_dev_commit_text_stage)");
  if (device_quals && s.host_quals) return fail(h, FEM_ERR_STATE, "BAM records need the qualities on the device (fem_dev_commit_text_stage, not _names_stage)");
  if (text && !h->d_ref_names) return fail(h, FEM_ERR_STATE, "reference names must be uploaded first (fem_dev_upload_reference_names)");
  s.prefetch_results = false;
  if (!s.tail) s.tail.reset(new (std::nothrow) femt::Tail());
  if (!s.tail) return fail(h, FEM_ERR_NOMEM, "out of host memory");
  f->in = tail_input(h, s);
  if (paired && (s.n_reads & 1)) return fail(h, FEM_ERR_INVALID, "a batch of read pairs holds an even number of reads");
  if (copy_records && s.out_stream) HIP_TRY(h, hipStreamSynchronize(s.out_stream));
  f->stream = copy_records ? s.stream : out_stream_of(h, s);
  std::string err;
  if ((rc = s.tail->run(f->in, f->stream, h->n_cu, h->tiny_buffers, &f->t, &err, h->timing ? f->ms : nullptr, copy_records))) return fail(h, rc, err);
  if (paired) {
    femt::RescueInput ri{};
    if ((rc = rescue_input(h, s, &ri))) return rc;
    if ((rc = s.tail->pair(s.min_insert, s.max_insert, f->stream, &err, s.rescue ? &ri : nullptr, s.mapq))) return fail(h, rc, err);
  }
  if (text) HIP_TRY(h, hipStreamWaitEvent(f->stream, s.ev_text_staged, 0));
  f->ms_run = since();
  if (copy_records && h->timing) {
    FEM_LOCK(h);
    for (int i = 0; i < 3; ++i) h->t_ms[3 + i] += f->ms[i], h->t_n[3 + i] += 1;
  }
  return FEM_OK;
}

static femt::SamInput sam_input(const fem_dev *h, const Slot &s) {
  return {s.host_quals ? nullptr : s.d_quals, s.d_names, s.d_name_off, h->d_ref_names, h->d_ref_name_off, s.host_quals, s.mapq, s.unmapped, s.report_strata, s.report_hits};
}

static int text_done(fem_dev *h, int slot, const TailFront &f, const char *tag, int id, const double *ms, int n_ms) {
  Slot &s = h->slot[slot];
  s.n_proper = s.paired ? s.tail->n_proper() : 0;
  s.n_rescued = s.paired ? s.tail->n_rescued() : 0;
  s.n_unmapped = s.tail->n_unmapped();
  s.n_filtered = s.tail->n_filtered();
  const bool report = s.report_strata >= 0 || s.report_hits >= 1;
  HIP_TRY(h, s.ev_text_order.create(hipEventDisableTiming));
  HIP_TRY(h, hipEventRecord(s.ev_text_order, f.stream));
  s.have_text_order = true;
  static const bool trace_host = testing_switch("FEM_FETCH_TIMES");
  if (trace_host) fprintf(stderr, "[%s] slot %d: mapping synced after %.2f ms, records %.2f, text sized and queued %.2f\n", tag, slot, f.ms_sync,
                          f.ms_run, std::chrono::duration<double, std::milli>(std::chrono::steady_clock::now() - f.t_in).count());
  if (h->timing) {
    FEM_LOCK(h);
    for (int i = 0; i < 3; ++i) h->t_ms[3 + i] += f.ms[i], h->t_n[3 + i] += 1;
    for (int i = 0; i < n_ms; ++i) h->t_ms[id + i] += ms[i], h->t_n[id + i] += 1;
    if (s.paired) h->t_ms[9] += s.tail->pair_ms(), h->t_n[9] += 1;
    if (s.paired && s.rescue) h->t_ms[10] += s.tail->rescue_ms(), h->t_n[10] += 1;
    if (s.mapq) h->t_ms[13] += s.tail->mapq_ms(), h->t_n[13] += 1;
    if (s.unmapped && !report) h->t_ms[14] += s.tail->unmapped_ms(), h->t_n[14] += 1;
    if (report) h->t_ms[15] += s.tail->report_ms(), h->t_n[15] += 1;
  }
  return FEM_OK;
}

int fem_dev_fetch_records(fem_dev *h, int slot, fem_batch_records *out) {
  TailFront f{};
  int rc = tail_records(h, slot, out, true, false, &f);
  if (rc) return rc;
  out->n_reads = f.t.n_reads, out->n_records = f.t.n_records;
  out->rec_begin = f.t.rec_begin, out->flag = f.t.flag, out->tid = f.t.tid, out->pos0 = f.t.pos0, out->nm = f.t.nm;
  out->cigar_off = f.t.cigar_off, out->cigar = f.t.cigar, out->md_off = f.t.md_off, out->md = f.t.md;
  memcpy(out->stats, h->slot[slot].stats, sizeof out->stats);
  return FEM_OK;
}

static int fetch_sam(fem_dev *h, int slot, fem_batch_sam *out, bool wait) {
  TailFront f{};
  int rc = tail_records(h, slot, out, false, false, &f);
  if (rc) return rc;
  Slot &s = h->slot[slot];
  femt::SamOutput text{};
  double ms_text = 0;
  std::string err;
  rc = s.tail->sam(f.in, sam_input(h, s), f.stream, h->n_cu, &text, &err, h->timing ? &ms_text : nullptr, wait, &h->text_gate, s.paired);
  if (rc) return fail(h, rc, err);
  if ((rc = text_done(h, slot, f, "fetch_sam", 7, &ms_text, wait ? 1 : 0))) return rc;
  s.qual_at = text.qual_at;
  out->text = text.text, out->len = text.len, out->n_asserted = text.n_asserted;
  out->n_reads = f.t.n_reads, out->n_records = f.t.n_records - s.n_filtered;
  memcpy(out->stats, s.stats, sizeof s.stats);
  return FEM_OK;
}

static int fetch_bam(fem_dev *h, int slot, int level, fem_batch_bam *out, bool wait) {
  if (level < 0 || level > 1) return fail(h, FEM_ERR_INVALID, "BAM compression level must be 0 or 1");
  TailFront f{};
  int rc = tail_records(h, slot, out, false, true, &f);
  if (rc) return rc;
  Slot &s = h->slot[slot];
  femt::BamOutput bam{};
  double ms_bam[2] = {0, 0};
// ... 426 lines not shown
```

### fem_amd/csrc/fem_kernels.hip.h

```cpp
#pragma once
#include <hip/hip_runtime.h>
#include <stdint.h>
#include "fem_planes.hip.h"

namespace femk {

constexpr int kWave = 64;
constexpr uint32_t kFlagCandOverflow = 1u;
constexpr uint32_t kFlagArenaOverflow = 2u;
constexpr uint32_t kFlagTooLarge = 4u;
constexpr uint32_t kInvalidMeta = 0xFFFFFFFFu;
constexpr int kMaxR = 10;
constexpr uint32_t kMeta16 = 0x80000000u;
constexpr uint32_t kSlotChunk = 256u;
constexpr uint32_t kFlagQueueOverflow = 8u;
constexpr uint32_t kQueueChunk = 32u;
constexpr uint32_t kInvalidRead = 0xFFFFFFFFu;

struct SeedLayout {
  uint32_t pkw, nkw;
  uint32_t sf;
  uint32_t dp_rows;
  uint32_t dp_bits;
  uint32_t picked;
  uint32_t rb;
  uint32_t X, F, A, B;
  uint32_t xcap, fcap, ccap;
  uint32_t smax, cmax, cw;
  uint32_t n_words;
  uint32_t blk, blk_bytes;
  uint32_t gq, gq_cap;
  uint32_t strm, strm_words;
  uint32_t fq, gstride, nb;
  uint32_t rinfo;
  uint32_t wave_bytes;
};

struct SeedParams {
  const uint8_t *bases;
  const uint64_t *read_off;
  uint32_t n_reads;
  uint32_t read_begin;
  uint32_t *work_cursor;
  const uint32_t *lookup;
  const uint64_t *occ;
  uint32_t inf32;
  const uint32_t *seq_len;
  int32_t e, a, R, k, step, lg;
  uint64_t *cand;
  uint32_t *cand_meta;
  uint32_t cand_cap;
  uint32_t *cand_begin;
  uint32_t *cand_count;
  uint32_t *ctr;
  uint32_t n_seq;
  uint32_t *slow_queue;
  uint32_t slow_cap;
  const uint32_t *work_queue;
  const uint32_t *summary;
  const uint32_t *occ32;
  uint32_t list_shift;
  const uint32_t *goff;
  const uint32_t *blkseq;
  const uint32_t *freq11;
  uint2 *sel;
  uint2 *sel_hdr;
  uint32_t n_banks;
  uint32_t bank_first[5];
  const uint32_t *bank_lo;
  uint32_t n_buckets;
  uint32_t blk_stride;
  unsigned long long *stats;
  uint64_t *arena;
  unsigned long long arena_cap;
  unsigned long long *arena_ctr;
  SeedLayout lay;
};

__global__ void uniform_offsets_kernel(uint64_t *off, uint64_t n, uint32_t len) {
  const uint64_t stride = (uint64_t)gridDim.x * blockDim.x;
  for (uint64_t i = (uint64_t)blockIdx.x * blockDim.x + threadIdx.x; i <= n; i += stride) off[i] = i * (uint64_t)len;
}

__global__ void unpack_reads_kernel(const uint8_t *packed, uint64_t n_reads, uint32_t len, uint32_t bytes_per_read, uint8_t *bases) {
  const uint64_t stride = (uint64_t)gridDim.x * blockDim.x, total = n_reads * bytes_per_read;
  const bool aligned = (len & 3u) == 0u && (((uintptr_t)bases) & 3u) == 0u;
  for (uint64_t i = (uint64_t)blockIdx.x * blockDim.x + threadIdx.x; i < total; i += stride) {
    const uint32_t b = packed[i];
    const uint32_t c0 = (0x54474341u >> (8u * (b & 3u))) & 0xFFu, c1 = (0x54474341u >> (8u * ((b >> 2) & 3u))) & 0xFFu;
    const uint32_t c2 = (0x54474341u >> (8u * ((b >> 4) & 3u))) & 0xFFu, c3 = (0x54474341u >> (8u * (b >> 6))) & 0xFFu;
    if (aligned) {
      ((uint32_t *)bases)[i] = c0 | (c1 << 8) | (c2 << 16) | (c3 << 24);
    } else {
      const uint64_t r = i / bytes_per_read;
      const uint32_t k = (uint32_t)(i - r * bytes_per_read) * 4u;
      uint8_t *o = bases + r * len + k;
      o[0] = (uint8_t)c0;
      if (k + 1u < len) o[1] = (uint8_t)c1;
      if (k + 2u < len) o[2] = (uint8_t)c2;
      if (k + 3u < len) o[3] = (uint8_t)c3;
    }
  }
}
__global__ void scatter_chars_kernel(const uint32_t *at, const uint8_t *ch, uint64_t n, uint8_t *bases) {
  const uint64_t stride = (uint64_t)gridDim.x * blockDim.x;
  for (uint64_t i = (uint64_t)blockIdx.x * blockDim.x + threadIdx.x; i < n; i += stride) bases[at[i]] = ch[i];
}

__global__ void mark_exception_reads_kernel(const uint32_t *at, uint64_t n, uint32_t len, uint32_t *bits) {
  const uint64_t stride = (uint64_t)gridDim.x * blockDim.x;
  for (uint64_t i = (uint64_t)blockIdx.x * blockDim.x + threadIdx.x; i < n; i += stride) {
    const uint32_t r = at[i] / len;
    atomicOr(&bits[r >> 5], 1u << (r & 31u));
  }
}

struct Picked {
  uint32_t start, lo, freq, pad;
};

struct Bufs {
  uint64_t *X;
  uint64_t *F;
  uint64_t *A;
  uint64_t *B;
  uint32_t xcap, fcap, ccap;
};

__device__ __forceinline__ uint32_t lane_id() { return threadIdx.x & 63u; }

#ifdef FEM_STAMPS
constexpr int kNumStamps = 12;
__device__ unsigned long long g_stamp_cycles[kNumStamps];
struct Prof {
  unsigned long long acc[kNumStamps] = {};
  unsigned long long last = 0;
  __device__ void start() { last = __builtin_amdgcn_s_memtime(); }
  __device__ void mark(int id) {
    unsigned long long t = __builtin_amdgcn_s_memtime();
    acc[id] += t - last;
    last = t;
  }
  __device__ void flush() {
    if (lane_id() == 0)
      for (int i = 0; i < kNumStamps; ++i) atomicAdd(&g_stamp_cycles[i], acc[i]);
  }
};
#define STAMP_START(p) (p).start()
#define STAMP(p, id) (p).mark(id)
#else
struct Prof {};
#define STAMP_START(p) ((void)0)
#define STAMP(p, id) ((void)0)
#endif

__device__ __forceinline__ void wave_sync_lds() {
  __builtin_amdgcn_fence(__ATOMIC_RELEASE, "wavefront");
  __builtin_amdgcn_wave_barrier();
  __builtin_amdgcn_fence(__ATOMIC_ACQUIRE, "wavefront");
}
__device__ __forceinline__ void wave_sync_global() {
  __builtin_amdgcn_fence(__ATOMIC_RELEASE, "workgroup");
  __builtin_amdgcn_wave_barrier();
  __builtin_amdgcn_fence(__ATOMIC_ACQUIRE, "workgroup");
}
template <bool GLOBAL>
__device__ __forceinline__ void wave_sync() {
  if (GLOBAL)
    wave_sync_global();
  else
    wave_sync_lds();
}

__device__ __forceinline__ uint32_t bcast0(uint32_t v) { return __builtin_amdgcn_readfirstlane(v); }

__device__ __forceinline__ uint32_t base_code(uint32_t c) {
  uint32_t x = (c >> 1) & 3u;
  uint32_t code = x ^ (x >> 1);
  uint32_t u = c & 0xDFu;
  bool acgt = (u == 'A') | (u == 'C') | (u == 'G') | (u == 'T');
  return acgt ? code : 4u;
}

__device__ __forceinline__ uint32_t reverse_pairs(uint32_t x, int k) {
  uint32_t r = __brev(x) >> (32 - 2 * k);
  return ((r & 0x55555555u) << 1) | ((r >> 1) & 0x55555555u);
}

template <typename T>
// ... 620 lines not shown
    uint32_t M = 0;
#pragma unroll
    for (int r = 1; r <= kUnroll; ++r) {
      if (r <= R) {
        const uint32_t v = M + f[r - 1];
        uint32_t x = in_seg ? v : inf;
        x = dpp_min_step<0x111, 0xF>(x, inf);
        x = dpp_min_step<0x112, 0xF>(x, inf);
        x = dpp_min_step<0x114, 0xF>(x, inf);
        x = dpp_min_step<0x118, 0xF>(x, inf);
        if (W > 16u) x = dpp_min_step<0x142, 0xA>(x, inf);
        if (W > 32u) x = dpp_min_step<0x143, 0xC>(x, inf);
        uint32_t ex = (uint32_t)__builtin_amdgcn_update_dpp((int)inf, (int)x, 0x138, 0xF, 0xF, false);
        ex = (c == 0 || ex > inf) ? inf : ex;
        const bool take = in_seg && v < ex;
        M = take ? v : ex;
        const unsigned long long bits = __ballot(take);
        if (ln == 0) take_bits[ps * (uint32_t)R + (uint32_t)(r - 1)] = bits;
      }
    }
    const uint32_t own_pass = ln / per_pass, own_slot = ln % per_pass;
    const uint32_t src = own_slot * W + (own_ncols ? own_ncols - 1u : 0u);
    const uint32_t got = __shfl(M, (int)src);
    if (ln < n_groups && own_pass == ps) pre_mine = got;
  }
  wave_sync_lds();
  if (ln < n_groups) {
    Picked *out = picked + (size_t)ln * (uint32_t)R;
    const uint32_t own_pass = ln / per_pass, own_slot = ln % per_pass;
    unsigned long long rows[kUnroll];
#pragma unroll
    for (int r = 1; r <= kUnroll; ++r) rows[r - 1] = (r <= R && own_ncols) ? take_bits[own_pass * (uint32_t)R + (uint32_t)(r - 1)] : 0ull;
    const uint2 *sfo = sf + (own_strand & 1u) * smax;
    int col = (int)own_ncols - 1, n_out = 0;
    bool alive = own_ncols != 0;
    uint32_t sidx[kUnroll];
#pragma unroll
    for (int r = kUnroll; r >= 1; --r) {
      sidx[r - 1] = 0xFFFFFFFFu;
      if (r <= R && alive) {
        unsigned long long seg = (rows[r - 1] >> (own_slot * W)) & ((2ull << col) - 1ull);
        if (seg == 0) {
          alive = false;
        } else {
          col = 63 - __builtin_clzll(seg);
          sidx[r - 1] = own_si + (uint32_t)step * (uint32_t)(col + (r - 1) * lg);
        }
      }
    }
#pragma unroll
    for (int r = kUnroll; r >= 1; --r) {
      if (r <= R) {
        Picked q{0, 0, 0, 0};
        if (sidx[r - 1] != 0xFFFFFFFFu) {
          uint2 s2 = sfo[sidx[r - 1]];
          q = Picked{sidx[r - 1], s2.x, s2.y, 0};
        }
        int slot_out = sidx[r - 1] != 0xFFFFFFFFu ? n_out++ : -1;
        if (slot_out >= 0) out[slot_out] = q;
      }
    }
    for (int t = n_out; t < R; ++t) out[t] = Picked{0, 0, 0, 0};
  }
  wave_sync_lds();
  {
    const uint32_t g = ln / (uint32_t)R, t = ln - g * (uint32_t)R;
    const bool act = ln < n_groups * (uint32_t)R;
    Picked mine{0, 0, 0, 0};
    uint32_t rank = 0;
    if (act) {
      const Picked *grp = picked + (size_t)g * (uint32_t)R;
      mine = grp[t];
      for (uint32_t u = 0; u < (uint32_t)R; ++u) {
        uint32_t fu = grp[u].freq;
        rank += (uint32_t)(fu < mine.freq || (fu == mine.freq && u < t));
      }
    }
    wave_sync_lds();
    if (act) picked[(size_t)g * (uint32_t)R + rank] = mine;
  }
  return pre_mine;
}

__global__ void __launch_bounds__(256) seed_filter_kernel(SeedParams p) {
  extern __shared__ __attribute__((aligned(16))) uint8_t smem[];
  const uint32_t ln = lane_id();
  const uint32_t wave_in_block = (uint32_t)__builtin_amdgcn_readfirstlane((int)(threadIdx.x >> 6));
  const uint32_t waves_per_block = blockDim.x >> 6;
  uint8_t *wbase = smem + (size_t)wave_in_block * p.lay.wave_bytes;
  uint32_t *pkw = (uint32_t *)(wbase + p.lay.pkw);
  uint32_t *nkw = (uint32_t *)(wbase + p.lay.nkw);
  uint2 *sf = (uint2 *)(wbase + p.lay.sf);
  uint32_t *dp_rows = (uint32_t *)(wbase + p.lay.dp_rows);
  uint32_t *dp_bits = (uint32_t *)(wbase + p.lay.dp_bits);
  Picked *picked = (Picked *)(wbase + p.lay.picked);
  uint32_t *rb = (uint32_t *)(wbase + p.lay.rb);
  Bufs lds;
  lds.X = (uint64_t *)(wbase + p.lay.X);
  lds.F = (uint64_t *)(wbase + p.lay.F);
  lds.A = (uint64_t *)(wbase + p.lay.A);
  lds.B = (uint64_t *)(wbase + p.lay.B);
  lds.xcap = p.lay.xcap, lds.fcap = p.lay.fcap, lds.ccap = p.lay.ccap;

  const int k = p.k, step = p.step, R = p.R, lg = p.lg;
  const uint32_t hash_mask = (k == 16) ? 0xFFFFFFFFu : ((1u << (2 * k)) - 1u);
  const uint32_t smax = p.lay.smax, cmax = p.lay.cmax, cw = p.lay.cw;
  unsigned long long pre_sum = 0, cand_sum = 0;
  SlotChunk chunk;
  Prof prof;

  const uint32_t wave_global = blockIdx.x * waves_per_block + wave_in_block;
  const uint32_t n_waves = gridDim.x * waves_per_block;

  const uint32_t n_items = p.work_queue ? min(p.ctr[2], p.slow_cap) : p.n_reads;
  for (uint32_t item = wave_global; item < n_items; item += n_waves) {
    const uint32_t read = p.work_queue ? p.work_queue[item] : item;
    if (read == kInvalidRead) continue;
    STAMP_START(prof);
    const uint64_t off = p.read_off[read];
    const uint32_t L = (uint32_t)(p.read_off[read + 1] - off);
    const uint8_t *seq = p.bases + off;
    const int S = (int)L - k + 1;

    bool shape_ok = S > 0 && R <= S / step;
    if (shape_ok) {
      int g_min = (S - (step - 1)) / step;
      shape_ok = g_min - R * lg + 2 >= 2;
    }
    if (!shape_ok || (uint32_t)S > smax) {
      if (ln < 2) {
        p.cand_begin[read * 2u + ln] = 0;
        p.cand_count[read * 2u + ln] = 0;
      }
      continue;
    }

    uint32_t n_fwd_amb = 0, n_rev_amb = 0;
    {
      const uint32_t n_words = (L + 15u) / 16u + 2u;
      for (uint32_t w = ln; w < n_words; w += kWave) {
        pkw[w] = 0;
        nkw[w] = 0;
      }
      wave_sync_lds();
      uint8_t *pkb = (uint8_t *)pkw, *nkb = (uint8_t *)nkw;
      for (uint32_t b0 = 0; b0 < L; b0 += 256u) {
        uint32_t idx = b0 + 4u * ln;
        if (idx < L) {
          uint32_t pv = 0, nv = 0;
#pragma unroll
          for (int q = 0; q < 4; ++q) {
            uint32_t c = 0, isn = 0;
            if (idx + q < L) {
              uint32_t code = base_code(seq[idx + q]);
              isn = code >> 2;
              c = code & 3u & (isn - 1u);
              n_fwd_amb += isn & (uint32_t)(idx + q >= (uint32_t)k);
              n_rev_amb += isn & (uint32_t)(L - 1u - (idx + q) >= (uint32_t)k);
            }
            pv = (pv << 2) | c;
            nv = (nv << 2) | (isn * 3u);
          }
          uint32_t byte_addr = (idx >> 4) * 4u + (3u - ((idx >> 2) & 3u));
          pkb[byte_addr] = (uint8_t)pv;
          nkb[byte_addr] = (uint8_t)nv;
        }
      }
      if (__any(n_fwd_amb | n_rev_amb)) {
        for (int d = 32; d >= 1; d >>= 1) {
          n_fwd_amb += __shfl_xor(n_fwd_amb, d);
          n_rev_amb += __shfl_xor(n_rev_amb, d);
        }
      }
      wave_sync_lds();
    }
    const bool strand_ok[2] = {n_fwd_amb <= (uint32_t)p.e, n_rev_amb <= (uint32_t)p.e};
    STAMP(prof, 0);

    for (int j0 = 0; j0 < S; j0 += kWave) {
      int j = j0 + (int)ln;
      if (j < S) {
        uint32_t w = (uint32_t)j >> 4, sh = 2u * ((uint32_t)j & 15u);
        uint64_t pw = ((uint64_t)pkw[w] << 32) | pkw[w + 1];
        uint64_t nw = ((uint64_t)nkw[w] << 32) | nkw[w + 1];
        uint32_t hf = (uint32_t)(pw >> (64 - 2 * k - sh)) & hash_mask;
        uint32_t nm = (uint32_t)(nw >> (64 - 2 * k - sh)) & hash_mask;
        uint32_t hr = reverse_pairs((~hf) & ~nm & hash_mask, k);
        if (strand_ok[0]) {
          uint32_t lo = p.lookup[hf], hi = p.lookup[hf + 1];
          sf[j] = make_uint2(lo, hi - lo);
        }
        if (strand_ok[1]) {
          uint32_t lo = p.lookup[hr], hi = p.lookup[hr + 1];
          sf[smax + (uint32_t)(S - 1 - j)] = make_uint2(lo, hi - lo);
        }
      }
    }
    wave_sync_lds();
    STAMP(prof, 1);

    uint32_t pre_g = 0;
    uint32_t dp_w = 0;
    if (2u * (uint32_t)step * (uint32_t)R <= (uint32_t)kWave && R <= kMaxR) {
      uint32_t widest = (uint32_t)(S / step - R * lg + 1);
      dp_w = widest <= 16u ? 16u : widest <= 32u ? 32u : widest <= 64u ? 64u : 0u;
    }
    if (dp_w) {
      pre_g = select_seeds_dpp<0, 0, 0>(p, S, strand_ok, sf, smax, dp_w, (unsigned long long *)dp_bits, picked);
    } else if (ln < 2u * (uint32_t)step && strand_ok[ln / (uint32_t)step]) {
      const uint32_t strand = ln / (uint32_t)step, si = ln % (uint32_t)step;
      const int G = (S - (int)si) / step;
      const int C = G - R * lg + 2;
      uint32_t *rows = dp_rows + (size_t)ln * 2u * cmax;
      uint32_t *bits = dp_bits + (size_t)ln * (uint32_t)R * cw;
      const uint2 *sfs = sf + strand * smax;
      for (int c = 1; c < C; ++c) rows[c] = 0;
      uint32_t left = p.inf32;
      for (int row = 1; row <= R; ++row) {
        const uint32_t *prev = rows + (size_t)((row - 1) & 1) * cmax;
        uint32_t *cur = rows + (size_t)(row & 1) * cmax;
        left = p.inf32;
        uint32_t acc = 0;
        for (int col = 1; col < C; ++col) {
          uint32_t pos = (uint32_t)(col + (row - 1) * lg - 1);
          uint32_t with_new = prev[col] + sfs[si + (uint32_t)step * pos].y;
          bool take = with_new < left;
          left = take ? with_new : left;
          cur[col] = left;
          acc |= (uint32_t)take << (col & 31);
          if ((col & 31) == 31 || col == C - 1) {
            bits[(uint32_t)(row - 1) * cw + ((uint32_t)col >> 5)] = acc;
            acc = 0;
          }
        }
      }
      pre_g = left;
      Picked *out = picked + (size_t)ln * (uint32_t)R;
// ... 227 lines not shown
```

### fem_amd/csrc/fem_seed_select.hip.h

```cpp
#pragma once
#include <type_traits>

#include "fem_seed_fast.hip.h"

namespace femk {

constexpr uint32_t kDenseMaxBanks = 4;
constexpr uint32_t kDenseNear = 1024u;
constexpr uint32_t kDenseRemap = 0xF0000000u;
constexpr uint32_t kSelKeepAll = 1u << 15;
constexpr uint32_t kSelOk = 0u, kSelNone = 1u, kSelSlow = 2u;
constexpr uint32_t kSelMaxCols = 128u;
constexpr uint32_t kSelMaxList = 128u;
constexpr uint32_t kX11 = 1u << 22;

__device__ __forceinline__ uint32_t wave_min_u32(uint32_t x) {
  constexpr uint32_t kFill = 0xFFFFFFFFu;
  x = dpp_min_step<0x111, 0xF>(x, kFill), x = dpp_min_step<0x112, 0xF>(x, kFill), x = dpp_min_step<0x114, 0xF>(x, kFill);
  x = dpp_min_step<0x118, 0xF>(x, kFill), x = dpp_min_step<0x142, 0xA>(x, kFill), x = dpp_min_step<0x143, 0xC>(x, kFill);
  return (uint32_t)__builtin_amdgcn_readlane((int)x, 63);
}
__device__ __forceinline__ uint32_t wave_max_u32(uint32_t x) {
  return (uint32_t)__builtin_amdgcn_readlane((int)wave_scan_max(x), 63);
}

__device__ __forceinline__ uint32_t rc11(uint32_t x) {
  const uint32_t r = __brev(~x & (kX11 - 1u)) >> 10;
  return ((r & 0x55555555u) << 1) | ((r >> 1) & 0x55555555u);
}

__global__ void freq11_kernel(const uint32_t *lookup, uint32_t *freq11) {
  const uint32_t stride = gridDim.x * blockDim.x;
  for (uint32_t t = blockIdx.x * blockDim.x + threadIdx.x; t < kX11 * 4u; t += stride) {
    const uint32_t X = t >> 2, i = t & 3u, rx = rc11(X);
    auto f = [&](uint32_t h) -> uint32_t {
      const uint32_t d = lookup[h + 1u] - lookup[h];
      return d < 255u ? d : 255u;
    };
    const uint32_t h_l = (i << 22) | X, h_r = (X << 2) | i;
    const uint32_t h_lrc = (rx << 2) | (3u - i), h_rrc = ((3u - i) << 22) | rx;
    freq11[t] = f(h_l) | (f(h_lrc) << 8) | (f(h_r) << 16) | (f(h_rrc) << 24);
  }
}

__device__ __forceinline__ uint32_t stream_window(const uint32_t *strm, uint32_t pos) {
  const uint32_t *w = strm + ((pos + 15u) >> 4) - 1;
  uint32_t twice = pos << 1;
  asm("" : "+v"(twice));
  return __builtin_amdgcn_alignbit(w[0], w[1], 0u - twice);
}
__device__ __forceinline__ uint32_t div3_small(uint32_t x) { return __umul24(x, 21846u) >> 16; }
__device__ __forceinline__ uint32_t div6_small(uint32_t x) { return __umul24(x, 10923u) >> 16; }
__device__ __forceinline__ uint32_t times3(uint32_t x) {
  uint32_t r;
  asm("v_lshl_add_u32 %0, %1, 1, %1" : "=v"(r) : "v"(x));
  return r;
}
__device__ __forceinline__ uint32_t rc_hash(uint32_t hf, uint32_t nm) {
  const uint32_t r = __brev((~hf) & ~nm & kHashMask) >> (32 - 2 * kK);
  return ((r & 0x55555555u) << 1) | ((r >> 1) & 0x55555555u);
}

template <int R, int W>
__device__ __forceinline__ void select_dp(const uint16_t *F, uint32_t ncols, uint32_t maxcols, uint32_t inf, uint32_t (&take)[R][W],
                                          uint32_t &m_last, uint32_t &iters) {
  uint32_t M[R];
#pragma unroll
  for (int r = 0; r < R; ++r) {
    M[r] = inf;
#pragma unroll
    for (int w = 0; w < W; ++w) take[r][w] = 0;
  }
  for (uint32_t c = 0; c < maxcols; ++c) {
    uint32_t f[R];
#pragma unroll
    for (int r = 0; r < R; ++r) f[r] = F[3u * c + 12u * (uint32_t)r];
    const bool in = c < ncols;
    uint32_t up = 0;
#pragma unroll
    for (int r = 0; r < R; ++r) {
      const uint32_t v = up + f[r];
      const bool tk = in && v < M[r];
      M[r] = tk ? v : M[r];
      up = M[r];
#pragma unroll
      for (int w = W - 1; w > 0; --w) take[r][w] = (take[r][w] << 1) | (take[r][w - 1] >> 31);
      take[r][0] = (take[r][0] << 1) | (uint32_t)tk;
    }
  }
  m_last = M[R - 1];
  iters = maxcols;
}
template <int W>
__device__ __forceinline__ int first_set_from(const uint32_t (&m)[W], uint32_t from) {
  int best = -1;
#pragma unroll
  for (int w = W - 1; w >= 0; --w) {
    const uint32_t lo = 32u * (uint32_t)w;
    uint32_t x = m[w];
    if (from > lo) x = from - lo >= 32u ? 0u : x & (0xFFFFFFFFu << (from - lo));
    if (x) best = (int)lo + __builtin_ctz(x);
  }
  return best;
}

#ifndef FEM_SELECT_WAVES
#define FEM_SELECT_WAVES 6
#endif
#ifndef FEM_SELECT_UNROLL
#define FEM_SELECT_UNROLL 2
#endif

template <int R, bool BANKED = false>
__global__ void __launch_bounds__(256) __attribute__((amdgpu_waves_per_eu(FEM_SELECT_WAVES, 8))) seed_select_kernel(SeedParams p) {
  extern __shared__ __attribute__((aligned(16))) uint8_t smem[];
  const uint32_t ln = lane_id();
  const uint32_t wave_in_block = (uint32_t)__builtin_amdgcn_readfirstlane((int)(threadIdx.x >> 6));
  uint8_t *wbase = smem + (size_t)wave_in_block * p.lay.wave_bytes;
  uint64_t *boff = (uint64_t *)(wbase + p.lay.rb);
  uint32_t *fw = (uint32_t *)(wbase + p.lay.strm);
  uint32_t *nw = fw + p.lay.strm_words;
  uint16_t *fq = (uint16_t *)(wbase + p.lay.fq);
  uint32_t *r_base = (uint32_t *)(wbase + p.lay.rinfo), *r_len = r_base + kReadBlock, *r_flag = r_len + kReadBlock,
           *r_pre = r_flag + kReadBlock;
  constexpr uint32_t kOk0 = 1u, kOk1 = 2u, kShape = 4u, kSlow = 8u;
  const uint32_t sstride = p.lay.gstride, nb = p.lay.nb;
  const uint32_t inf = p.inf32;
  SlotChunk qchunk;

  auto queue_slow = [&](uint32_t read) {
    if (qchunk.left == 0) {
      uint32_t base = 0;
      if (ln == 0) base = atomicAdd(&p.ctr[2], kQueueChunk);
      qchunk.next = bcast0(base);
      qchunk.left = kQueueChunk;
    }
    if (qchunk.next < p.slow_cap) {
      if (ln == 0) p.slow_queue[qchunk.next] = read;
    } else if (ln == 0) {
      atomicOr(&p.ctr[1], kFlagQueueOverflow);
    }
    ++qchunk.next, --qchunk.left;
  };

  for (;;) {
    uint32_t pull = 0;
    if (ln == 0) pull = atomicAdd(p.work_cursor, kReadBlock);
    pull = bcast0(pull);
    if ((uint64_t)p.read_begin + pull >= p.n_reads) break;
    const uint32_t r0 = p.read_begin + pull;
    const uint32_t n_blk = p.n_reads - r0 < kReadBlock ? p.n_reads - r0 : kReadBlock;
    wave_sync_lds();
    if (ln <= n_blk) boff[ln] = p.read_off[r0 + ln];
    wave_sync_lds();
    for (uint32_t sb = 0; sb < n_blk; sb += nb) {
      const uint32_t cnt = n_blk - sb < nb ? n_blk - sb : nb;
      const uint32_t rd0 = r0 + sb;
      const uint64_t o_first = boff[sb];
      const uint64_t blk_off = (uint64_t)__builtin_amdgcn_readfirstlane((uint32_t)o_first) |
                               ((uint64_t)__builtin_amdgcn_readfirstlane((uint32_t)(o_first >> 32)) << 32);
      uint32_t my_S = 0, my_flag = 0;
      {
        uint32_t L = 0, base = 0;
        if (ln < cnt) {
          const uint64_t o0 = boff[sb + ln], o1 = boff[sb + ln + 1u];
          L = (uint32_t)(o1 - o0), base = (uint32_t)(o0 - blk_off);
          const int S = (int)L - kK + 1;
          bool shape_ok = S > 0 && R <= S / kStep;
          if (shape_ok) shape_ok = (S - (kStep - 1)) / kStep - R * kLg + 2 >= 2;
          if (shape_ok) {
            my_S = (uint32_t)S;
            my_flag = kShape | kOk0 | kOk1;
            const uint32_t widest = (uint32_t)(S / kStep - R * kLg + 1);
            if (widest > kSelMaxCols || p.a == 0) my_flag |= kSlow;
          }
        }
        if (ln < kReadBlock) r_base[ln] = base, r_len[ln] = L, r_flag[ln] = my_flag, r_pre[ln] = 0;
      }
      const uint32_t total_chars = (uint32_t)(boff[sb + cnt] - blk_off);
      uint32_t any_n = 0;
      {
        const uint8_t *src = p.bases + blk_off;
        for (uint32_t q = ln; 4u * q < total_chars; q += (uint32_t)kWave) {
          uint32_t code, nflag;
          encode4(load_u32_unaligned(src + 4u * q), code, nflag);
          const uint32_t left = total_chars - 4u * q;
          const uint32_t keep = left >= 4u ? 0xFFFFFFFFu : ((1u << (8u * left)) - 1u);
          nflag &= keep;
          code &= keep & ~(nflag * 3u);
          const uint32_t byte_addr = (q >> 2) * 4u + (3u - (q & 3u));
          ((uint8_t *)fw)[byte_addr] = (uint8_t)pack4(code);
          ((uint8_t *)nw)[byte_addr] = (uint8_t)pack4(nflag * 3u);
          any_n |= nflag;
        }
      }
      const bool has_n = __builtin_amdgcn_ballot_w64(any_n != 0) != 0;
      wave_sync_lds();
      if (has_n) {
        for (uint32_t i = 0; i < cnt; ++i) {
          const uint32_t L = r_len[i], base = r_base[i];
          uint32_t n_f = 0, n_r = 0;
          for (uint32_t b0 = 0; b0 < L; b0 += (uint32_t)kWave) {
            const uint32_t at = b0 + ln;
            if (at < L) {
              const uint32_t pos = base + at;
              const uint32_t isn = (nw[pos >> 4] >> (30u - 2u * (pos & 15u))) & 1u;
              n_f += isn & (uint32_t)(at >= (uint32_t)kK);
              n_r += isn & (uint32_t)(L - 1u - at >= (uint32_t)kK);
            }
          }
          for (int d = 32; d >= 1; d >>= 1) n_f += __shfl_xor(n_f, d), n_r += __shfl_xor(n_r, d);
          if (ln == 0) {
            uint32_t fl = r_flag[i];
            if (n_f > (uint32_t)p.e) fl &= ~kOk0;
            if (n_r > (uint32_t)p.e) fl &= ~kOk1;
            r_flag[i] = fl;
          }
        }
        wave_sync_lds();
      }
      const uint32_t SP = wave_max_u32(my_S);
      if (SP != 0) {
        const uint32_t SPp = (SP + 1u) >> 1;
        const uint32_t magic = 0xFFFFFFFFu / SPp + 1u;
        const uint32_t total = cnt * SPp;
        constexpr int U = FEM_SELECT_UNROLL;
        constexpr uint32_t kActBit = 1u << 25, kTwoBit = 1u << 24;
        for (uint32_t w0 = 0; w0 < total; w0 += (uint32_t)(U * kWave)) {
          uint32_t d0[U], d1[U], where[U];
#pragma unroll
          for (int u = 0; u < U; ++u) {
            const uint32_t w = w0 + (uint32_t)(u * kWave) + ln;
            const uint32_t i = __umulhi(w, magic);
            const uint32_t j = (w - __umul24(i, SPp)) << 1;
            const uint32_t i_c = i < cnt ? i : 0u;
            const uint32_t fl = r_flag[i_c];
            const uint32_t S = r_len[i_c] - (uint32_t)(kK - 1);
            const bool act = w < total && (fl & kShape) && !(fl & kSlow) && j < S;
            const bool two = act && j + 1u < S;
            const uint32_t win = stream_window(fw, act ? r_base[i_c] + j : 0u);
            const uint32_t hf0 = win >> 8;
            const uint32_t at0 = ((hf0 & (kX11 - 1u)) << 2) | (hf0 >> 22), at1 = (win >> 6) & kHashMask;
            d0[u] = p.freq11[act ? at0 : 0u];
            d1[u] = p.freq11[two ? at1 : 0u];
            where[u] = i_c | (j << 4) | (S << 14) | (two ? kTwoBit : 0u) | (act ? kActBit : 0u);
          }
#pragma unroll
          for (int u = 0; u < U; ++u) {
            if (where[u] & kActBit) {
              const uint32_t i = where[u] & 15u, j = (where[u] >> 4) & 1023u, S = (where[u] >> 14) & 1023u;
              const bool two = (where[u] & kTwoBit) != 0u;
              uint32_t x = (d0[u] & 0x0000FFFFu) | (d1[u] & 0xFFFF0000u);
              if (!two) x &= 0x0000FFFFu;
              uint32_t ffwd = x & 0x00FF00FFu, frev = (x >> 8) & 0x00FF00FFu;
              const uint32_t is255 = ((x & 0x7F7F7F7Fu) + 0x01010101u) & x & 0x80808080u;
              if (has_n || is255 != 0u) {
                uint32_t f2[2] = {0u, 0u}, r2[2] = {0u, 0u};
#pragma unroll
                for (int q = 0; q < 2; ++q) {
                  if (q == 1 && !two) continue;
                  uint32_t f_fwd = (x >> (16 * q)) & 255u, f_rev = (x >> (16 * q + 8)) & 255u;
                  const uint32_t pos = r_base[i] + j + (uint32_t)q;
                  const uint32_t hf = stream_window(fw, pos) >> 8;
                  const uint32_t nm = has_n ? stream_window(nw, pos) >> 8 : 0u;
// ... 156 lines not shown
```

### fem_amd/device.py

```python
import ctypes as C
import os

import numpy as np

_HERE = os.path.dirname(os.path.abspath(__file__))
_HIP = None

ABI_SYMBOLS = [
    "fem_dev_open", "fem_dev_close", "fem_strerror", "fem_dev_last_error", "fem_dev_limits",
    "fem_dev_upload_index", "fem_dev_upload_reference", "fem_dev_build_index", "fem_dev_fetch_index",
    "fem_dev_map_batch_submit", "fem_dev_map_batch_wait",
    "fem_dev_stage_reads", "fem_dev_stage_info", "fem_dev_acquire_stage", "fem_dev_commit_stage", "fem_dev_commit_stage_uniform", "fem_dev_packed_layout", "fem_dev_commit_stage_packed", "fem_dev_map_staged", "fem_dev_sync", "fem_dev_fetch_stats", "fem_dev_fetch", "fem_dev_fetch_packed",
    "fem_dev_fetch_records", "fem_dev_seed_kernel", "fem_dev_index_info",
    "fem_dev_upload_reference_names", "fem_dev_acquire_text_stage", "fem_dev_commit_text_stage", "fem_dev_commit_names_stage", "fem_dev_sam_quals", "fem_dev_reserve_text", "fem_dev_reserve_batch", "fem_set_blocking_waits", "fem_dev_fetch_sam", "fem_dev_fetch_sam_nowait", "fem_dev_sam_wait",
    "fem_dev_set_timing", "fem_dev_reset_timing", "fem_dev_kernel_time", "fem_dev_copy_bandwidth",
    "fem_dev_h2d_bandwidth", "fem_dbg_live_bytes",
    "fem_device_numa", "fem_bind_thread_near_device",
    "fem_dev_allreduce_stats",
    "fem_dev_set_pairs", "fem_dev_fetch_pairs", "fem_dev_pair_count",
    "fem_dev_set_rescue", "fem_dev_rescue_count", "fem_dev_set_mapq",
    "fem_dev_set_unmapped", "fem_dev_unmapped_count",
    "fem_dev_set_report", "fem_dev_filtered_count",
    "fem_dev_fetch_bam", "fem_dev_fetch_bam_nowait", "fem_dev_bam_wait", "fem_dev_bgzf_compress",
]


class FemError(RuntimeError):
    pass


class Params(C.Structure):
    _fields_ = [("k", C.c_int32), ("step", C.c_int32), ("e", C.c_int32), ("a", C.c_int32)]


class _ReadBatch(C.Structure):
    _fields_ = [("bases", C.c_void_p), ("offsets", C.c_void_p), ("n_reads", C.c_uint64)]


class _BatchResult(C.Structure):
    _fields_ = [("n_reads", C.c_uint64), ("n_candidates", C.c_uint64), ("cand_begin", C.c_void_p),
                ("cand_count", C.c_void_p), ("cand", C.c_void_p), ("ed", C.c_void_p), ("end", C.c_void_p),
                ("stats", C.c_uint64 * 5)]


class _BatchPacked(C.Structure):
    _fields_ = [("n_reads", C.c_uint64), ("n_candidates", C.c_uint64), ("count", C.c_void_p), ("seg_begin", C.c_void_p),
                ("cand", C.c_void_p), ("ed", C.c_void_p), ("end", C.c_void_p), ("big", C.c_void_p), ("n_big", C.c_uint32),
                ("stats", C.c_uint64 * 5)]


class _BatchRecords(C.Structure):
    _fields_ = [("n_reads", C.c_uint64), ("n_records", C.c_uint64), ("rec_begin", C.c_void_p), ("flag", C.c_void_p),
                ("tid", C.c_void_p), ("pos0", C.c_void_p), ("nm", C.c_void_p), ("cigar_off", C.c_void_p),
                ("cigar", C.c_void_p), ("md_off", C.c_void_p), ("md", C.c_void_p), ("stats", C.c_uint64 * 5)]


class _BatchSam(C.Structure):
    _fields_ = [("text", C.c_void_p), ("len", C.c_uint64), ("n_reads", C.c_uint64), ("n_records", C.c_uint64),
                ("n_asserted", C.c_uint64), ("stats", C.c_uint64 * 5)]


class _BatchBam(C.Structure):
    _fields_ = [("data", C.c_void_p), ("len", C.c_uint64), ("raw_len", C.c_uint64), ("n_blocks", C.c_uint64),
                ("n_records", C.c_uint64), ("n_asserted", C.c_uint64), ("stats", C.c_uint64 * 5)]


class _PairParams(C.Structure):
    _fields_ = [("min_insert", C.c_int32), ("max_insert", C.c_int32)]


class _RescueParams(C.Structure):
    _fields_ = [("max_edits", C.c_int32)]


class _ReportParams(C.Structure):
    _fields_ = [("strata", C.c_int32), ("max_hits", C.c_int32)]


class _BatchPairs(C.Structure):
    _fields_ = [("n_pairs", C.c_uint64), ("n_records", C.c_uint64), ("rec_begin", C.c_void_p), ("flag", C.c_void_p),
                ("tid", C.c_void_p), ("pos0", C.c_void_p), ("nm", C.c_void_p), ("cigar_off", C.c_void_p),
                ("cigar", C.c_void_p), ("md_off", C.c_void_p), ("md", C.c_void_p), ("mate_tid", C.c_void_p),
                ("mate_pos0", C.c_void_p), ("tlen", C.c_void_p), ("n_proper", C.c_uint64), ("stats", C.c_uint64 * 5)]


def hip_library_path():
    return os.environ.get("FEM_HIP_LIBRARY") or os.path.join(_HERE, "csrc", "libfemhip.so")


def load_hip():
    global _HIP
    if _HIP is not None:
        return _HIP
    path = hip_library_path()
    if not os.path.exists(path):
        raise FemError("libfemhip.so is missing (%s): run `python -c 'import __graft_entry__ as g; g.build()'` "
                       "or `make -C fem_amd/csrc`" % path)
    L = C.CDLL(path)
    vp, u64, i32 = C.c_void_p, C.c_uint64, C.c_int32
    L.fem_dev_open.argtypes = [C.c_int, C.POINTER(vp)]
    L.fem_dev_close.argtypes = [vp]
    L.fem_strerror.restype = C.c_char_p
    L.fem_strerror.argtypes = [C.c_int]
    L.fem_dev_last_error.restype = C.c_char_p
    L.fem_dev_last_error.argtypes = [vp]
    L.fem_dev_limits.argtypes = [vp, C.POINTER(C.c_uint32), C.POINTER(i32)]
    L.fem_dev_upload_index.argtypes = [vp, i32, i32, vp, u64, vp, u64]
    L.fem_dev_upload_reference.argtypes = [vp, C.c_uint32, C.POINTER(vp), vp]
    L.fem_dev_build_index.argtypes = [vp, i32, i32, vp, vp, u64, C.POINTER(u64)]
    L.fem_dev_fetch_index.argtypes = [vp, vp, vp, u64]
    L.fem_dev_map_batch_submit.argtypes = [vp, C.c_int, C.POINTER(Params), C.POINTER(_ReadBatch)]
    L.fem_dev_map_batch_wait.argtypes = [vp, C.c_int, C.POINTER(_BatchResult)]
    L.fem_dev_stage_reads.argtypes = [vp, C.c_int, C.POINTER(_ReadBatch)]
    L.fem_dev_acquire_stage.argtypes = [vp, C.c_int, u64, u64, C.POINTER(vp), C.POINTER(vp)]
    L.fem_dev_commit_stage.argtypes = [vp, C.c_int, u64, C.c_uint32]
    L.fem_dev_commit_stage_uniform.argtypes = [vp, C.c_int, u64, C.c_uint32]
    L.fem_dev_packed_layout.argtypes = [u64, C.c_uint32, C.POINTER(C.c_uint32), C.POINTER(u64), C.POINTER(u64)]
    L.fem_dev_commit_stage_packed.argtypes = [vp, C.c_int, u64, C.c_uint32, u64]
    L.fem_dev_map_staged.argtypes = [vp, C.c_int, C.POINTER(Params)]
    L.fem_dev_sync.argtypes = [vp, C.c_int]
    L.fem_dev_fetch_stats.argtypes = [vp, C.c_int, vp]
    L.fem_dev_fetch.argtypes = [vp, C.c_int, C.POINTER(_BatchResult)]
    L.fem_dev_fetch_packed.argtypes = [vp, C.c_int, C.POINTER(_BatchPacked)]
    L.fem_dev_fetch_records.argtypes = [vp, C.c_int, C.POINTER(_BatchRecords)]
    L.fem_dev_index_info.argtypes = [vp, C.c_char_p, u64]
    L.fem_dev_seed_kernel.restype = C.c_char_p
    L.fem_dev_seed_kernel.argtypes = [vp, C.POINTER(Params)]
    L.fem_dev_set_timing.argtypes = [vp, C.c_int]
    L.fem_dev_reset_timing.argtypes = [vp]
    L.fem_dev_kernel_time.argtypes = [vp, C.c_int, C.POINTER(C.c_double), C.POINTER(u64)]
    L.fem_dev_copy_bandwidth.argtypes = [vp, u64, C.c_int, C.POINTER(C.c_double)]
    L.fem_dev_h2d_bandwidth.argtypes = [vp, u64, C.c_int, C.POINTER(C.c_double)]
    L.fem_dev_allreduce_stats.argtypes = [C.POINTER(vp), C.c_int, vp]
    L.fem_dev_upload_reference_names.argtypes = [vp, C.c_uint32, C.c_char_p, vp]
    L.fem_dev_acquire_text_stage.argtypes = [vp, C.c_int, u64, u64, u64, C.POINTER(vp), C.POINTER(vp), C.POINTER(vp)]
    L.fem_dev_commit_text_stage.argtypes = [vp, C.c_int, u64, u64]
    if hasattr(L, "fem_dev_commit_names_stage"):
        L.fem_dev_commit_names_stage.argtypes = [vp, C.c_int, u64, u64]
        L.fem_dev_sam_quals.argtypes = [vp, C.c_int, C.POINTER(vp), C.POINTER(u64)]
    L.fem_dev_reserve_text.argtypes = [vp, C.c_int, u64, u64, u64, u64]
    if hasattr(L, "fem_dev_reserve_batch"):
        L.fem_dev_reserve_batch.argtypes = [vp, C.c_int, u64, u64, C.c_uint32, C.POINTER(Params)]
    L.fem_dev_fetch_sam.argtypes = [vp, C.c_int, C.POINTER(_BatchSam)]
    L.fem_dev_fetch_sam_nowait.argtypes = [vp, C.c_int, C.POINTER(_BatchSam)]
    L.fem_dev_sam_wait.argtypes = [vp, C.c_int]
    L.fem_dev_stage_info.argtypes = [vp, C.c_int, C.POINTER(u64), C.POINTER(C.c_int32)]
    if hasattr(L, "fem_dev_set_pairs"):
        L.fem_dev_set_pairs.argtypes = [vp, C.c_int, C.POINTER(_PairParams)]
        L.fem_dev_fetch_pairs.argtypes = [vp, C.c_int, C.POINTER(_BatchPairs)]
        L.fem_dev_pair_count.argtypes = [vp, C.c_int, C.POINTER(u64)]
    if hasattr(L, "fem_dev_set_rescue"):
        L.fem_dev_set_rescue.argtypes = [vp, C.c_int, C.POINTER(_RescueParams)]
        L.fem_dev_rescue_count.argtypes = [vp, C.c_int, C.POINTER(u64)]
    if hasattr(L, "fem_dev_set_mapq"):
        L.fem_dev_set_mapq.argtypes = [vp, C.c_int, C.c_int]
    if hasattr(L, "fem_dev_set_unmapped"):
        L.fem_dev_set_unmapped.argtypes = [vp, C.c_int, C.c_int]
        L.fem_dev_unmapped_count.argtypes = [vp, C.c_int, C.POINTER(u64)]
    if hasattr(L, "fem_dev_set_report"):
        L.fem_dev_set_report.argtypes = [vp, C.c_int, C.POINTER(_ReportParams)]
        L.fem_dev_filtered_count.argtypes = [vp, C.c_int, C.POINTER(u64)]
    if hasattr(L, "fem_dev_fetch_bam"):
        L.fem_dev_fetch_bam.argtypes = [vp, C.c_int, C.c_int, C.POINTER(_BatchBam)]
        L.fem_dev_fetch_bam_nowait.argtypes = [vp, C.c_int, C.c_int, C.POINTER(_BatchBam)]
        L.fem_dev_bam_wait.argtypes = [vp, C.c_int]
        L.fem_dev_bgzf_compress.argtypes = [vp, vp, u64, C.c_int, vp, u64, C.POINTER(u64)]
    if hasattr(L, "fem_dbg_live_bytes"):
        L.fem_dbg_live_bytes.argtypes = [C.POINTER(u64), C.POINTER(u64)]
    L.fem_device_numa.argtypes = [C.c_int, C.POINTER(C.c_int32), C.c_char_p, u64]
    L.fem_bind_thread_near_device.argtypes = [C.c_int]
    _HIP = L
    return L


def device_numa(device=0):
    node = C.c_int32(-1)
    buf = C.create_string_buffer(4096)
    rc = load_hip().fem_device_numa(int(device), C.byref(node), buf, 4096)
    if rc != 0:
        raise FemError("fem_device_numa: %d" % rc)
    return node.value, buf.value.decode()


def bind_near_device(device=0):
    return load_hip().fem_bind_thread_near_device(int(device)) == 0


def live_bytes():
    dev, pin = C.c_uint64(), C.c_uint64()
    rc = load_hip().fem_dbg_live_bytes(C.byref(dev), C.byref(pin))
    if rc != 0:
        raise FemError("fem_dbg_live_bytes: %d" % rc)
    return dev.value, pin.value


def packed_layout(n_reads, read_len):
    bpr, off, cap = C.c_uint32(), C.c_uint64(), C.c_uint64()
    rc = load_hip().fem_dev_packed_layout(int(n_reads), int(read_len), C.byref(bpr), C.byref(off), C.byref(cap))
    if rc != 0:
        raise FemError("fem_dev_packed_layout: %d" % rc)
    return bpr.value, off.value, cap.value


def pack_reads(bases, n_reads, read_len, out):
    bpr, exc_off, exc_cap = packed_layout(n_reads, read_len)
    b = np.asarray(bases[:n_reads * read_len], dtype=np.uint8).reshape(n_reads, read_len)
    ok = (b == 65) | (b == 67) | (b == 71) | (b == 84)
    code = np.where(ok, ((b >> 1) ^ (b >> 2)) & 3, 0).astype(np.uint8)
    pad = bpr * 4 - read_len
    if pad:
        code = np.concatenate([code, np.zeros((n_reads, pad), np.uint8)], axis=1)
    q = code.reshape(n_reads, bpr, 4)
    out[:n_reads * bpr] = (q[:, :, 0] | (q[:, :, 1] << 2) | (q[:, :, 2] << 4) | (q[:, :, 3] << 6)).reshape(-1)
    out[n_reads * bpr:exc_off] = 0
    pos = np.flatnonzero(~ok.reshape(-1)).astype(np.uint32)
    n_exc = len(pos)
    if n_exc > exc_cap:
        raise FemError("too many exceptions for a packed batch")
    out[exc_off:exc_off + 4 * n_exc] = pos.view(np.uint8)
    out[exc_off + 4 * n_exc:exc_off + 5 * n_exc] = b.reshape(-1)[pos]
    return n_exc


def _copy(ptr, n, dtype, copy=True):
    n = int(n)
    if n == 0 or not ptr:
        return np.zeros(0, dtype=dtype)
    buf = (C.c_char * (n * np.dtype(dtype).itemsize)).from_address(ptr)
    a = np.frombuffer(buf, dtype=dtype, count=n)
# ... 98 lines not shown
        self.md = _copy(r.md, int(self.md_off[-1]), np.uint8)
        self.mate_tid = _copy(r.mate_tid, nr, np.uint32)
        self.mate_pos0 = _copy(r.mate_pos0, nr, np.uint32)
        self.tlen = _copy(r.tlen, nr, np.int32)
        self.stats = np.array(list(r.stats), dtype=np.uint64)


class Device:

    def __init__(self, device=0):
        self._L = load_hip()
        h = C.c_void_p()
        rc = self._L.fem_dev_open(device, C.byref(h))
        if rc != 0:
            raise FemError("fem_dev_open(%d) failed: %s — the HIP path needs a GPU, there is no CPU fallback"
                           % (device, self._L.fem_strerror(rc).decode()))
        self._h = h
        self._keep = []

    def close(self):
        if self._h:
            self._L.fem_dev_close(self._h)
            self._h = None

    def __del__(self):
        try:
            self.close()
        except Exception:
            pass

    def _check(self, rc):
        if rc != 0:
            raise FemError("%s: %s" % (self._L.fem_strerror(rc).decode(),
                                       self._L.fem_dev_last_error(self._h).decode()))

    def limits(self):
        m, s = C.c_uint32(), C.c_int32()
        self._check(self._L.fem_dev_limits(self._h, C.byref(m), C.byref(s)))
        return m.value, s.value

    def upload_index(self, k, step, lookup, occ, n_occ=None):
        lookup = np.ascontiguousarray(lookup, dtype=np.uint32)
        occ = np.ascontiguousarray(occ, dtype=np.uint64)
        n_occ = len(occ) if n_occ is None else n_occ
        self._check(self._L.fem_dev_upload_index(self._h, k, step, lookup.ctypes.data, len(lookup), occ.ctypes.data,
                                                 n_occ))

    def upload_reference(self, seqs):
        arrs = [np.frombuffer(s, dtype=np.uint8) if isinstance(s, (bytes, bytearray)) else np.ascontiguousarray(s, np.uint8)
                for s in seqs]
        ptrs = (C.c_void_p * len(arrs))(*[a.ctypes.data for a in arrs])
        lens = np.array([len(a) for a in arrs], dtype=np.uint32)
        self._check(self._L.fem_dev_upload_reference(self._h, len(arrs), ptrs, lens.ctypes.data))

    def build_index(self, k=12, step=3, fetch=True):
        n = C.c_uint64()
        self._check(self._L.fem_dev_build_index(self._h, k, step, None, None, 0, C.byref(n)))
        if not fetch:
            return int(n.value), None, None
        lookup, occ = self.fetch_index(k, int(n.value))
        return int(n.value), lookup, occ

    def fetch_index(self, k, n_occ):
        lookup = np.zeros((1 << (2 * k)) + 1, dtype=np.uint32)
        occ = np.zeros(max(int(n_occ), 1), dtype=np.uint64)
        self._check(self._L.fem_dev_fetch_index(self._h, lookup.ctypes.data, occ.ctypes.data, len(occ)))
        return lookup, occ[:int(n_occ)]

    @staticmethod
    def _batch(bases, offsets):
        bases = np.ascontiguousarray(bases, dtype=np.uint8)
        offsets = np.ascontiguousarray(offsets, dtype=np.uint64)
        return _ReadBatch(bases.ctypes.data, offsets.ctypes.data, len(offsets) - 1), (bases, offsets)

    def stage_reads(self, bases, offsets, slot=0):
        b, keep = self._batch(bases, offsets)
        self._check(self._L.fem_dev_stage_reads(self._h, slot, C.byref(b)))

    def stage_info(self, slot=0):
        nb, pk = C.c_uint64(0), C.c_int32(0)
        self._check(self._L.fem_dev_stage_info(self._h, slot, C.byref(nb), C.byref(pk)))
        return nb.value, bool(pk.value)

    def acquire_stage(self, n_reads_cap, n_bases_cap, slot=0):
        pb, po = C.c_void_p(), C.c_void_p()
        self._check(self._L.fem_dev_acquire_stage(self._h, slot, n_reads_cap, n_bases_cap, C.byref(pb), C.byref(po)))
        bases = np.frombuffer((C.c_char * (int(n_bases_cap) + 64)).from_address(pb.value), dtype=np.uint8)
        offs = np.frombuffer((C.c_char * (8 * (int(n_reads_cap) + 1))).from_address(po.value), dtype=np.uint64)
        return bases, offs

    def commit_stage(self, n_reads, max_len, slot=0, uniform=False):
        if uniform:
            self._check(self._L.fem_dev_commit_stage_uniform(self._h, slot, n_reads, max_len))
        else:
            self._check(self._L.fem_dev_commit_stage(self._h, slot, n_reads, max_len))

    def commit_stage_packed(self, n_reads, read_len, n_exc=0, slot=0):
        self._check(self._L.fem_dev_commit_stage_packed(self._h, slot, n_reads, read_len, n_exc))

    def map_staged(self, e=3, a=1, k=12, step=3, slot=0):
        p = Params(k, step, e, a)
        self._check(self._L.fem_dev_map_staged(self._h, slot, C.byref(p)))

    def sync(self, slot=0):
        self._check(self._L.fem_dev_sync(self._h, slot))

    def fetch_stats(self, slot=0):
        st = np.zeros(5, dtype=np.uint64)
        self._check(self._L.fem_dev_fetch_stats(self._h, slot, st.ctypes.data))
        return st

    def fetch(self, slot=0, copy=True):
        r = _BatchResult()
        self._check(self._L.fem_dev_fetch(self._h, slot, C.byref(r)))
        return BatchResult(r, copy)

    def fetch_packed(self, slot=0, copy=True):
        r = _BatchPacked()
        self._check(self._L.fem_dev_fetch_packed(self._h, slot, C.byref(r)))
        return BatchPacked(r, copy)

    def seed_kernel(self, e=3, a=1, k=12, step=3):
        p = Params(k, step, e, a)
        return self._L.fem_dev_seed_kernel(self._h, C.byref(p)).decode()

    def index_info(self):
        buf = C.create_string_buffer(512)
        self._check(self._L.fem_dev_index_info(self._h, buf, 512))
        return buf.value.decode()

    def reserve_batch(self, n_reads, n_records, max_len, e=3, a=1, k=12, step=3, slot=0):
        p = Params(k, step, e, a)
        self._check(self._L.fem_dev_reserve_batch(self._h, slot, n_reads, n_records, max_len, C.byref(p)))

    def fetch_records(self, slot=0):
        r = _BatchRecords()
        self._check(self._L.fem_dev_fetch_records(self._h, slot, C.byref(r)))
        return BatchRecords(r)

    def upload_reference_names(self, names):
        raw = [n.encode() if isinstance(n, str) else bytes(n) for n in names]
        off = np.zeros(len(raw) + 1, np.uint64)
        off[1:] = np.cumsum([len(n) for n in raw])
        self._check(self._L.fem_dev_upload_reference_names(self._h, len(raw), b"".join(raw), off.ctypes.data))

    def stage_text(self, quals, names, slot=0, quals_on_host=False):
        raw = [n.encode() if isinstance(n, str) else bytes(n) for n in names]
        q = np.frombuffer(bytes(quals), np.uint8) if not isinstance(quals, np.ndarray) else quals
        nn = sum(len(n) for n in raw)
        pq, pn, po = C.c_void_p(), C.c_void_p(), C.c_void_p()
        self._check(self._L.fem_dev_acquire_text_stage(self._h, slot, len(raw), len(q), nn, C.byref(pq), C.byref(pn), C.byref(po)))
        if len(q):
            C.memmove(pq.value, q.ctypes.data, len(q))
        if nn:
            C.memmove(pn.value, b"".join(raw), nn)
        off = np.zeros(len(raw) + 1, np.uint64)
        off[1:] = np.cumsum([len(n) for n in raw])
        C.memmove(po.value, off.ctypes.data, 8 * (len(raw) + 1))
        if quals_on_host:
            self._check(self._L.fem_dev_commit_names_stage(self._h, slot, len(raw), nn))
        else:
            self._check(self._L.fem_dev_commit_text_stage(self._h, slot, len(raw), nn))

    def fetch_sam(self, slot=0, nowait=False, quals=None, offsets=None):
        r = _BatchSam()
        if nowait:
# ... 119 lines not shown
```

### include/fem_hip.h

```cpp
#ifndef FEM_HIP_H_
#define FEM_HIP_H_

#include <stddef.h>
#include <stdint.h>

#ifdef __cplusplus
extern "C" {
#endif

enum fem_status {
  FEM_OK = 0,
  FEM_ERR_INVALID = -1,
  FEM_ERR_HIP = -2,
  FEM_ERR_NOMEM = -3,
  FEM_ERR_STATE = -4,
  FEM_ERR_UNSUPPORTED = -5,
  FEM_ERR_RCCL = -6
};

typedef struct {
  int32_t k;
  int32_t step;
  int32_t e;
  int32_t a;
} fem_params;

typedef struct {
  const char *bases;
  const uint64_t *offsets;
  uint64_t n_reads;
} fem_read_batch;

typedef struct {
  uint64_t n_reads;
  uint64_t n_candidates;
  const uint32_t *cand_begin;
  const uint32_t *cand_count;
  const uint64_t *cand;
  const uint8_t *ed;
  const int16_t *end;
  uint64_t stats[5];
} fem_batch_result;

typedef struct {
  uint64_t n_reads;
  uint64_t n_candidates;
  const uint8_t *count;
  const uint32_t *seg_begin;
  const uint64_t *cand;
  const uint8_t *ed;
  const int16_t *end;
  const uint32_t *big;
  uint32_t n_big;
  uint64_t stats[5];
} fem_batch_packed;

typedef struct {
  uint64_t n_reads;
  uint64_t n_records;
  const uint32_t *rec_begin;
  const uint16_t *flag;
  const uint32_t *tid;
  const uint32_t *pos0;
  const uint8_t *nm;
  const uint32_t *cigar_off;
  const uint32_t *cigar;
  const uint32_t *md_off;
  const char *md;
  uint64_t stats[5];
} fem_batch_records;

typedef struct {
  const char *text;
  uint64_t len;
  uint64_t n_reads, n_records;
  uint64_t n_asserted;
  uint64_t stats[5];
} fem_batch_sam;

typedef struct fem_dev fem_dev;

int fem_set_blocking_waits(int on);

int fem_dev_open(int device, fem_dev **out);
int fem_dev_close(fem_dev *h);
const char *fem_strerror(int rc);
const char *fem_dev_last_error(const fem_dev *h);
int fem_dev_limits(const fem_dev *h, uint32_t *max_read_len, int32_t *n_slots);

int fem_dev_upload_index(fem_dev *h, int32_t k, int32_t step, const uint32_t *lookup, uint64_t n_lookup,
                         const uint64_t *occ, uint64_t n_occ);
int fem_dev_upload_reference(fem_dev *h, uint32_t n_seq, const char *const *seq, const uint32_t *seq_len);
int fem_dev_build_index(fem_dev *h, int32_t k, int32_t step, uint32_t *lookup_out, uint64_t *occ_out,
                        uint64_t occ_cap, uint64_t *n_occ_out);
int fem_dev_fetch_index(fem_dev *h, uint32_t *lookup_out, uint64_t *occ_out, uint64_t occ_cap);

int fem_dev_map_batch_submit(fem_dev *h, int slot, const fem_params *p, const fem_read_batch *reads);
int fem_dev_map_batch_wait(fem_dev *h, int slot, fem_batch_result *out);

int fem_dev_stage_reads(fem_dev *h, int slot, const fem_read_batch *reads);
int fem_dev_stage_info(fem_dev *h, int slot, uint64_t *h2d_bytes, int32_t *packed);
int fem_dev_acquire_stage(fem_dev *h, int slot, uint64_t n_reads_cap, uint64_t n_bases_cap, char **bases,
                          uint64_t **offsets);
int fem_dev_commit_stage(fem_dev *h, int slot, uint64_t n_reads, uint32_t max_len);
int fem_dev_commit_stage_uniform(fem_dev *h, int slot, uint64_t n_reads, uint32_t read_len);
int fem_dev_packed_layout(uint64_t n_reads, uint32_t read_len, uint32_t *bytes_per_read, uint64_t *exc_offset, uint64_t *exc_cap);
int fem_dev_commit_stage_packed(fem_dev *h, int slot, uint64_t n_reads, uint32_t read_len, uint64_t n_exceptions);
int fem_dev_map_staged(fem_dev *h, int slot, const fem_params *p);
int fem_dev_sync(fem_dev *h, int slot);
int fem_dev_fetch_stats(fem_dev *h, int slot, uint64_t stats[5]);
int fem_dev_fetch(fem_dev *h, int slot, fem_batch_result *out);
int fem_dev_fetch_packed(fem_dev *h, int slot, fem_batch_packed *out);
int fem_dev_fetch_records(fem_dev *h, int slot, fem_batch_records *out);

int fem_dev_upload_reference_names(fem_dev *h, uint32_t n_seq, const char *names, const uint64_t *name_off);
int fem_dev_acquire_text_stage(fem_dev *h, int slot, uint64_t n_reads_cap, uint64_t n_bases_cap, uint64_t n_name_bytes_cap,
                               char **quals, char **names, uint64_t **name_off);
int fem_dev_commit_text_stage(fem_dev *h, int slot, uint64_t n_reads, uint64_t n_name_bytes);
int fem_dev_commit_names_stage(fem_dev *h, int slot, uint64_t n_reads, uint64_t n_name_bytes);
int fem_dev_sam_quals(fem_dev *h, int slot, const uint64_t **qual_at, uint64_t *n_reads);
int fem_dev_reserve_text(fem_dev *h, int slot, uint64_t n_reads, uint64_t n_bases, uint64_t n_name_bytes, uint64_t text_bytes);
int fem_dev_reserve_batch(fem_dev *h, int slot, uint64_t n_reads, uint64_t n_records, uint32_t max_len, const fem_params *p);
int fem_dev_fetch_sam(fem_dev *h, int slot, fem_batch_sam *out);
int fem_dev_fetch_sam_nowait(fem_dev *h, int slot, fem_batch_sam *out);
int fem_dev_sam_wait(fem_dev *h, int slot);

typedef struct {
  const uint8_t *data;
  uint64_t len, raw_len, n_blocks, n_records, n_asserted;
  uint64_t stats[5];
} fem_batch_bam;
int fem_dev_fetch_bam(fem_dev *h, int slot, int level, fem_batch_bam *out);
int fem_dev_fetch_bam_nowait(fem_dev *h, int slot, int level, fem_batch_bam *out);
int fem_dev_bam_wait(fem_dev *h, int slot);
int fem_dev_bgzf_compress(fem_dev *h, const void *in, uint64_t n, int level, void *out, uint64_t out_cap, uint64_t *out_len);

typedef struct {
  int32_t min_insert, max_insert;
} fem_pair_params;
int fem_dev_set_pairs(fem_dev *h, int slot, const fem_pair_params *pp);
typedef struct {
  uint64_t n_pairs, n_records;
  const uint32_t *rec_begin;
  const uint16_t *flag;
  const uint32_t *tid, *pos0;
  const uint8_t *nm;
  const uint32_t *cigar_off, *cigar, *md_off;
  const char *md;
  const uint32_t *mate_tid, *mate_pos0;
  const int32_t *tlen;
  uint64_t n_proper;
  uint64_t stats[5];
} fem_batch_pairs;
int fem_dev_fetch_pairs(fem_dev *h, int slot, fem_batch_pairs *out);
int fem_dev_pair_count(fem_dev *h, int slot, uint64_t *n_proper);

#define FEM_RESCUE_ANCHORS 8
typedef struct {
  int32_t max_edits;
} fem_rescue_params;
int fem_dev_set_rescue(fem_dev *h, int slot, const fem_rescue_params *rp);
int fem_dev_rescue_count(fem_dev *h, int slot, uint64_t *n_rescued);

int fem_dev_set_mapq(fem_dev *h, int slot, int on);

int fem_dev_set_unmapped(fem_dev *h, int slot, int on);
int fem_dev_unmapped_count(fem_dev *h, int slot, uint64_t *n);

typedef struct {
  int32_t strata;
  int32_t max_hits;
} fem_report_params;
int fem_dev_set_report(fem_dev *h, int slot, const fem_report_params *rp);
int fem_dev_filtered_count(fem_dev *h, int slot, uint64_t *n);

const char *fem_dev_seed_kernel(const fem_dev *h, const fem_params *p);
int fem_dev_index_info(const fem_dev *h, char *buf, uint64_t cap);

int fem_dev_set_timing(fem_dev *h, int on);
int fem_dev_reset_timing(fem_dev *h);
int fem_dev_kernel_time(fem_dev *h, int kernel, double *ms_total, uint64_t *launches);
int fem_dev_copy_bandwidth(fem_dev *h, uint64_t bytes, int iters, double *gb_per_s);
int fem_dev_h2d_bandwidth(fem_dev *h, uint64_t bytes, int iters, double *gb_per_s);
int fem_dbg_live_bytes(uint64_t *device_bytes, uint64_t *pinned_bytes);
// ... 11 lines not shown
```

Baseline: 393.1.

## Feed seed select kernel directly from 2-bit packed reads, defer full unpack

When reads arrive packed and the dense seeding path is used, the select kernel now reads the 2-bit codes directly from the packed buffer, converting them into its forward words in LDS. Only reads containing exception characters are unpacked to byte bases at commit. The full unpack of all reads to byte bases, and the offsets kernel, are deferred until a later stage needs them, via ensure_chars and an event. The aim is to skip writing and re-reading the full byte-per-base array before seeding. The cost is an extra kernel template variant, more state flags, and the tail stage now triggering the deferred unpack on its own stream.

```diff
diff --git a/fem_amd/csrc/fem_hip.hip b/fem_amd/csrc/fem_hip.hip
--- a/fem_amd/csrc/fem_hip.hip
+++ b/fem_amd/csrc/fem_hip.hip
@@ -51,6 +51,7 @@
 constexpr uint32_t kMaxReadLen = 1024;
 constexpr size_t kFrontPad = 16;
 constexpr size_t kPackedFrontPad = 256;
+constexpr uint64_t kExpandAllShare = 8;
 constexpr uint32_t kXcapSmall = 512, kFcap = 128, kCcap = 128;
 
 constexpr int kTimedKernels = 16;
@@ -93,6 +94,9 @@
   uint64_t prefetched_reads2 = 0, prefetched_cand = 0, last_n_cand = 0;
   uint64_t h2d_bytes = 0;
   bool sent_packed = false;
+  bool chars_ready = true, offs_ready = true, select_packed = false;
+  uint64_t n_exc = 0;
+  Event ev_chars;
   int parts = 1;
   uint32_t part_begin[kMaxParts + 1] = {0, 0, 0, 0, 0};
   Event ev_part[kMaxParts], ev_sel[kMaxParts];
@@ -240,6 +244,7 @@
   Buf<uint32_t> d_occ32, d_goff, d_blkseq;
   uint32_t list_shift = 0;
   bool no_strided = false;
+  bool select_chars = false;
   bool verify_chars = false;
   Buf<uint32_t> d_freq11;
   uint32_t n_banks = 1, bank_first[5] = {0, 0, 0, 0, 0};
@@ -393,7 +398,7 @@
   return l;
 }
 
-femk::SeedLayout make_layout_select(const fem_params &p, uint32_t max_len) {
+femk::SeedLayout make_layout_select(const fem_params &p, uint32_t max_len, bool packed) {
   femk::SeedLayout l{};
   const uint32_t R = (uint32_t)(p.e + 1 + p.a);
   l.smax = max_len >= (uint32_t)p.k ? max_len - (uint32_t)p.k + 1u : 1u;
@@ -402,7 +407,7 @@
   l.gstride += l.gstride & 1u;
   if (!((l.gstride >> 1) & 1u)) l.gstride += 2u;
   l.nb = std::max<uint32_t>(1u, std::min<uint32_t>(femk::kReadBlock, 3100u / (2u * 2u * l.gstride)));
-  l.strm_words = (l.nb * max_len + 15u) / 16u + 2u;
+  l.strm_words = (l.nb * (packed ? (max_len + 3u) & ~3u : max_len) + 15u) / 16u + 2u;
   uint32_t o = 0;
   auto take = [&](uint32_t bytes) {
     uint32_t at = o;
@@ -439,16 +444,18 @@
 
 typedef void (*SeedKernel)(femk::SeedParams);
 template <size_t... I>
-SeedKernel select_kernel_of(int R, bool banked, std::index_sequence<I...>) {
-  static const SeedKernel k[2][femk::kMaxR] = {{femk::seed_select_kernel<(int)I + 1, false>...}, {femk::seed_select_kernel<(int)I + 1, true>...}};
-  return k[banked][std::min(std::max(R, 1), femk::kMaxR) - 1];
+SeedKernel select_kernel_of(int R, bool banked, bool packed, std::index_sequence<I...>) {
+  static const SeedKernel k[2][2][femk::kMaxR] = {
+      {{femk::seed_select_kernel<(int)I + 1, false, false>...}, {femk::seed_select_kernel<(int)I + 1, true, false>...}},
+      {{femk::seed_select_kernel<(int)I + 1, false, true>...}, {femk::seed_select_kernel<(int)I + 1, true, true>...}}};
+  return k[packed][banked][std::min(std::max(R, 1), femk::kMaxR) - 1];
 }
 template <size_t... I>
 SeedKernel fast_kernel_of(int R, bool hash, std::index_sequence<I...>) {
   static const SeedKernel k[2][femk::kMaxR] = {{femk::seed_fast_kernel<(int)I + 1, false>...}, {femk::seed_fast_kernel<(int)I + 1, true>...}};
   return k[hash][std::min(std::max(R, 1), femk::kMaxR) - 1];
 }
-SeedKernel select_kernel(int R, bool banked) { return select_kernel_of(R, banked, std::make_index_sequence<femk::kMaxR>{}); }
+SeedKernel select_kernel(int R, bool banked, bool packed) { return select_kernel_of(R, banked, packed, std::make_index_sequence<femk::kMaxR>{}); }
 SeedKernel fast_kernel(int R, bool hash) { return fast_kernel_of(R, hash, std::make_index_sequence<femk::kMaxR>{}); }
 SeedKernel join_kernel(int R, int which) {
   static const SeedKernel k[3][femk::kMaxR] = {
@@ -467,19 +474,19 @@
   int nb = 0;
   return hipOccupancyMaxActiveBlocksPerMultiprocessor(&nb, kernel, block, lds) == hipSuccess ? nb : 0;
 }
-uint32_t kernel_regs(int R, bool join, int which = 0) {
-  static std::atomic<uint32_t> cache[3][2][femk::kMaxR + 1] = {};
-  std::atomic<uint32_t> &slot = cache[which][join ? 1 : 0][std::min(std::max(R, 1), femk::kMaxR)];
+uint32_t kernel_regs(int R, bool join, int which = 0, bool packed = false) {
+  static std::atomic<uint32_t> cache[3][3][femk::kMaxR + 1] = {};
+  std::atomic<uint32_t> &slot = cache[which][join ? 1 : packed ? 2 : 0][std::min(std::max(R, 1), femk::kMaxR)];
   uint32_t c = slot.load(std::memory_order_relaxed);
   if (c) return c;
   hipFuncAttributes a{};
-  const void *f = join ? (const void *)join_kernel(R, which) : (const void *)select_kernel(R, which == 1);
+  const void *f = join ? (const void *)join_kernel(R, which) : (const void *)select_kernel(R, which == 1, packed);
   c = hipFuncGetAttributes(&a, f) == hipSuccess && a.numRegs > 0 ? (uint32_t)a.numRegs : 128u;
   slot.store(c, std::memory_order_relaxed);
   return c;
 }
 void launch_select(int R, bool banked, dim3 grid, dim3 block, uint32_t lds, hipStream_t st, const femk::SeedParams &sp) {
-  hipLaunchKernelGGL(select_kernel(R, banked), grid, block, lds, st, sp);
+  hipLaunchKernelGGL(select_kernel(R, banked, sp.packed != nullptr), grid, block, lds, st, sp);
 }
 void launch_join(int R, int which, dim3 grid, dim3 block, uint32_t lds, hipStream_t st, const femk::SeedParams &sp) {
   hipLaunchKernelGGL(join_kernel(R, which), grid, block, lds, st, sp);
@@ -650,6 +657,8 @@
   return FEM_OK;
 }
 
+int ensure_chars(fem_dev *h, Slot &s);
+
 int launch_batch(fem_dev *h, Slot &s) {
   const fem_params &p = s.params;
   uint32_t *d_ctr = (uint32_t *)s.d_ctl.get();
@@ -676,7 +685,18 @@
     HIP_TRY(h, hipMemsetAsync(s.d_ctl, 0, kCtlAlloc, s.stream));
   }
 
+  const int R_all = p.e + 1 + p.a;
+  const bool dense_kernels = !h->force_generic && p.k == femk::kK && p.step == femk::kStep && R_all >= 1 && R_all <= femk::kMaxR && h->d_occ32 && h->d_freq11;
+  if (s.n_reads && (!dense_kernels || h->verify_chars)) {
+    int rc = ensure_chars(h, s);
+    if (rc) return rc;
+  }
   femk::SeedParams sp{};
+  s.select_packed = false;
+  if (s.sent_packed && !h->select_chars && dense_kernels) {
+    sp.packed = s.packed(), sp.exc_bits = s.d_exc_bits, sp.bpr = s.packed_bpr, sp.len = s.max_len;
+    s.select_packed = s.n_reads != 0;
+  }
   sp.bases = s.bases();
   sp.read_off = s.d_off;
   sp.n_reads = (uint32_t)s.n_reads;
@@ -748,7 +768,7 @@
       fp.blk_stride = (femk::kDenseRemap >> femk::kDenseBlkShift) + 1u;
       for (uint32_t b = 0; b <= femk::kDenseMaxBanks; ++b) fp.bank_first[b] = h->bank_first[b];
       uint32_t select_lds = 0, select_threads = 256;
-      fp.lay = make_layout_select(p, max_len);
+      fp.lay = make_layout_select(p, max_len, fp.packed != nullptr);
       if (fp.lay.wave_bytes > 64u * 1024u) return fail(h, FEM_ERR_UNSUPPORTED, "read too long for the device path");
       const femk::SeedLayout lay_select = fp.lay;
       femk::SeedLayout lay_join = make_layout_join(p, banked, !banked && h->list_shift != 0);
@@ -760,8 +780,9 @@
       uint64_t per_cu_s, per_cu_j;
       {
         const uint32_t lds_bytes = wpb_s * lay_select.wave_bytes;
-        const uint64_t key = ((uint64_t)banked << 48) | ((uint64_t)R << 40) | lds_bytes;
-        if (h->select_occ_key != key) h->select_occ_key = key, h->select_occ_blocks = blocks_per_cu((const void *)select_kernel(R, banked), (int)(64u * wpb_s), lds_bytes);
+        const uint64_t key = ((uint64_t)(fp.packed != nullptr) << 49) | ((uint64_t)banked << 48) | ((uint64_t)R << 40) | lds_bytes;
+        if (h->select_occ_key != key)
+          h->select_occ_key = key, h->select_occ_blocks = blocks_per_cu((const void *)select_kernel(R, banked, fp.packed != nullptr), (int)(64u * wpb_s), lds_bytes);
         per_cu_s = h->select_occ_blocks > 0 ? (uint64_t)h->select_occ_blocks : std::max<uint64_t>(1, 160u * 1024u / lds_bytes);
         if (overlap) per_cu_s = 1;
         select_lds = lds_bytes, select_threads = 64u * wpb_s;
@@ -771,7 +792,7 @@
         if (h->join_occ_key != key) h->join_occ_key = key, h->join_occ_blocks = blocks_per_cu((const void *)join_kernel(R, which), (int)(64u * wpb_j), lds_j);
         per_cu_j = h->join_occ_blocks > 0 ? (uint64_t)h->join_occ_blocks : std::max<uint64_t>(1, 160u * 1024u / lds_j);
         if (overlap) {
-          const uint32_t vj = (kernel_regs(R, true, which) + 7u) & ~7u, vs = (kernel_regs(R, false, banked ? 1 : 0) + 7u) & ~7u;
+          const uint32_t vj = (kernel_regs(R, true, which) + 7u) & ~7u, vs = (kernel_regs(R, false, banked ? 1 : 0, fp.packed != nullptr) + 7u) & ~7u;
           const uint32_t wj = 64u * wpb_j / 256u ? 64u * wpb_j / 256u : 1u, ws = select_threads / 256u ? select_threads / 256u : 1u;
           const uint32_t lj = (lds_j + 511u) & ~511u, ls = (select_lds + 511u) & ~511u;
           while (per_cu_j > 1 && (per_cu_j * wj * vj + ws * vs > 512u || per_cu_j * lj + ls > 160u * 1024u || per_cu_j * wj + ws > 8u)) --per_cu_j;
@@ -1026,6 +1047,29 @@
 
 using fempack::pack_bases;
 
+int ensure_chars(fem_dev *h, Slot &s) {
+  if (s.chars_ready) return FEM_OK;
+  const uint64_t n = s.n_reads, n_exc = s.n_exc;
+  const uint32_t len = s.max_len, bpr = s.packed_bpr;
+  const uint64_t code_bytes = fempack::code_bytes(n, len);
+  if (!s.offs_ready)
+    hipLaunchKernelGGL(femk::uniform_offsets_kernel, dim3((uint32_t)std::min<uint64_t>((n + 256) / 256, (uint64_t)h->n_cu * 8u)), dim3(256), 0,
+                       s.stream, s.d_off, n, len);
+  if (n) {
+    const uint32_t grid = (uint32_t)std::min<uint64_t>((n * bpr + 255) / 256, (uint64_t)h->n_cu * 16u);
+    hipLaunchKernelGGL(femk::unpack_reads_kernel, dim3(grid), dim3(256), 0, s.stream, (const uint8_t *)s.packed(), n, len, bpr, s.bases());
+  }
+  if (n_exc) {
+    const dim3 g((uint32_t)std::min<uint64_t>((n_exc + 255) / 256, (uint64_t)h->n_cu * 4u));
+    hipLaunchKernelGGL(femk::scatter_chars_kernel, g, dim3(256), 0, s.stream, (const uint32_t *)(s.packed() + code_bytes),
+                       (const uint8_t *)(s.packed() + code_bytes + 4u * n_exc), n_exc, s.bases());
+  }
+  HIP_TRY(h, hipGetLastError());
+  HIP_TRY(h, hipEventRecord(s.ev_chars, s.stream));
+  s.chars_ready = true, s.offs_ready = true;
+  return FEM_OK;
+}
+
 int enqueue_packed(fem_dev *h, Slot &s, uint64_t n, uint32_t len, uint64_t n_exc) {
   const uint32_t bpr = fempack::bytes_per_read(len);
   const uint64_t code_bytes = fempack::code_bytes(n, len), n_bases = n * (uint64_t)len;
@@ -1040,8 +1084,11 @@
     s.parts = (int)std::min<uint64_t>((uint64_t)h->max_parts, n / kPartMinReads);
   for (int q = 0; q <= s.parts; ++q) s.part_begin[q] = q == s.parts ? (uint32_t)n : (uint32_t)((n * q / s.parts) & ~63ull);
   HIP_TRY(h, hipMemsetAsync(s.d_exc_bits, 0, ((size_t)n / 32 + 1) * sizeof(uint32_t), s.stream));
-  hipLaunchKernelGGL(femk::uniform_offsets_kernel, dim3((uint32_t)std::min<uint64_t>((n + 256) / 256, (uint64_t)h->n_cu * 8u)), dim3(256), 0,
-                     s.stream, s.d_off, n, len);
+  const bool at_commit = h->select_chars || n_exc * kExpandAllShare > n;
+  const bool offs_at_commit = at_commit || !(h->d_occ32 && h->d_freq11);
+  if (offs_at_commit)
+    hipLaunchKernelGGL(femk::uniform_offsets_kernel, dim3((uint32_t)std::min<uint64_t>((n + 256) / 256, (uint64_t)h->n_cu * 8u)), dim3(256), 0,
+                       s.stream, s.d_off, n, len);
   if ((rc = h2d_begin(h, s))) return rc;
   for (int q = 0; q < s.parts; ++q) {
     const uint64_t r0 = s.part_begin[q], r1 = s.part_begin[q + 1];
@@ -1049,7 +1096,7 @@
     Span span(h, s, 20, s.stream);
     if (b1 > b0) HIP_TRY(h, hipMemcpyAsync(s.packed() + b0, s.h_bases + b0, b1 - b0, hipMemcpyHostToDevice, s.stream));
     if (q + 1 == s.parts && (rc = h2d_end(h, s))) return rc;
-    if (r1 > r0) {
+    if (at_commit && r1 > r0) {
       const uint32_t grid = (uint32_t)std::min<uint64_t>(((r1 - r0) * bpr + 255) / 256, (uint64_t)h->n_cu * 16u);
       hipLaunchKernelGGL(femk::unpack_reads_kernel, dim3(grid), dim3(256), 0, s.stream, (const uint8_t *)s.packed() + b0, r1 - r0, len, bpr,
                          s.bases() + r0 * len);
@@ -1058,6 +1105,11 @@
   }
   if (n_exc) {
     const dim3 g((uint32_t)std::min<uint64_t>((n_exc + 255) / 256, (uint64_t)h->n_cu * 4u));
+    if (!at_commit) {
+      const dim3 gm((uint32_t)std::min<uint64_t>((n_exc * bpr + 255) / 256, (uint64_t)h->n_cu * 8u));
+      hipLaunchKernelGGL(femk::unpack_marked_reads_kernel, gm, dim3(256), 0, s.stream, (const uint8_t *)s.packed(),
+                         (const uint32_t *)(s.packed() + code_bytes), n_exc, len, bpr, s.bases(), s.d_off.get());
+    }
     hipLaunchKernelGGL(femk::scatter_chars_kernel, g, dim3(256), 0, s.stream, (const uint32_t *)(s.packed() + code_bytes),
                        (const uint8_t *)(s.packed() + code_bytes + 4u * n_exc), n_exc, s.bases());
     hipLaunchKernelGGL(femk::mark_exception_reads_kernel, g, dim3(256), 0, s.stream, (const uint32_t *)(s.packed() + code_bytes), n_exc, len,
@@ -1068,6 +1120,7 @@
   s.n_reads = n, s.n_bases = n_bases, s.max_len = len;
   s.staged = true, s.mapped = false, s.synced = false;
   s.h2d_bytes = total, s.sent_packed = true;
+  s.chars_ready = at_commit, s.offs_ready = offs_at_commit, s.n_exc = n_exc;
   return FEM_OK;
 }
 
@@ -1130,7 +1183,7 @@
   for (int i = 0; ok_ev && i < kSlots; ++i) {
     Slot &sl = h->slot[i];
     ok_ev = sl.ev_zeroed.create(hipEventDisableTiming) == hipSuccess && sl.ev_results.create(hipEventDisableTiming) == hipSuccess &&
-            sl.ev_home.create(hipEventDisableTiming) == hipSuccess;
+            sl.ev_home.create(hipEventDisableTiming) == hipSuccess && sl.ev_chars.create(hipEventDisableTiming) == hipSuccess;
     for (int q = 0; ok_ev && q < kMaxParts; ++q)
       ok_ev = sl.ev_part[q].create(hipEventDisableTiming) == hipSuccess && sl.ev_sel[q].create(hipEventDisableTiming) == hipSuccess;
   }
@@ -1151,6 +1204,7 @@
     h->no_dense = testing_switch("FEM_NO_DENSE");
     h->no_strided = testing_switch("FEM_NO_STRIDED");
     h->verify_chars = testing_switch("FEM_VERIFY_CHARS");
+    h->select_chars = testing_switch("FEM_SELECT_CHARS");
     h->tiny_buffers = testing_switch("FEM_TEST_TINY_BUFFERS");
     if (const char *bl = getenv("FEM_TEST_BANK_BASES")) h->bank_limit = strtoull(bl, nullptr, 10);
     if (const char *bs = getenv("FEM_TEST_BANK_SEQS")) h->bank_seqs = (uint32_t)strtoul(bs, nullptr, 10);
@@ -1337,7 +1391,7 @@
   s.parts = 1;
   s.n_reads = n_reads, s.n_bases = n_bases, s.max_len = max_len;
   s.staged = true, s.mapped = false, s.synced = false;
-  s.h2d_bytes = n_bases + (n_reads ? (n_reads + 1) * sizeof(uint64_t) : 0), s.sent_packed = false, s.staged_by_copy = false;
+  s.h2d_bytes = n_bases + (n_reads ? (n_reads + 1) * sizeof(uint64_t) : 0), s.sent_packed = false, s.chars_ready = true, s.offs_ready = true, s.n_exc = 0, s.staged_by_copy = false;
   return FEM_OK;
 }
 
@@ -1363,7 +1417,7 @@
   HIP_TRY(h, hipGetLastError());
   s.n_reads = n_reads, s.n_bases = n_bases, s.max_len = read_len;
   s.staged = true, s.mapped = false, s.synced = false;
-  s.h2d_bytes = n_bases, s.sent_packed = false, s.staged_by_copy = false;
+  s.h2d_bytes = n_bases, s.sent_packed = false, s.chars_ready = true, s.offs_ready = true, s.n_exc = 0, s.staged_by_copy = false;
   return FEM_OK;
 }
 
@@ -1498,6 +1552,14 @@
   return FEM_OK;
 }
 
+int fem_dev_stage_front(fem_dev *h, int slot, int32_t *select_packed, int32_t *chars_ready) {
+  int rc = check_slot(h, slot);
+  if (rc) return rc;
+  if (select_packed) *select_packed = h->slot[slot].select_packed ? 1 : 0;
+  if (chars_ready) *chars_ready = h->slot[slot].chars_ready ? 1 : 0;
+  return FEM_OK;
+}
+
 int fem_dev_map_staged(fem_dev *h, int slot, const fem_params *p) {
   int rc = check_slot(h, slot);
   if (rc) return rc;
@@ -1872,6 +1934,8 @@
   if (paired && (s.n_reads & 1)) return fail(h, FEM_ERR_INVALID, "a batch of read pairs holds an even number of reads");
   if (copy_records && s.out_stream) HIP_TRY(h, hipStreamSynchronize(s.out_stream));
   f->stream = copy_records ? s.stream : out_stream_of(h, s);
+  if ((rc = ensure_chars(h, s))) return rc;
+  if (s.sent_packed && f->stream != s.stream.s) HIP_TRY(h, hipStreamWaitEvent(f->stream, s.ev_chars, 0));
   std::string err;
   if ((rc = s.tail->run(f->in, f->stream, h->n_cu, h->tiny_buffers, &f->t, &err, h->timing ? f->ms : nullptr, copy_records))) return fail(h, rc, err);
   if (paired) {
diff --git a/fem_amd/csrc/fem_kernels.hip.h b/fem_amd/csrc/fem_kernels.hip.h
--- a/fem_amd/csrc/fem_kernels.hip.h
+++ b/fem_amd/csrc/fem_kernels.hip.h
@@ -75,6 +75,9 @@
   unsigned long long arena_cap;
   unsigned long long *arena_ctr;
   SeedLayout lay;
+  const uint8_t *packed;
+  const uint32_t *exc_bits;
+  uint32_t bpr, len;
 };
 
 __global__ void uniform_offsets_kernel(uint64_t *off, uint64_t n, uint32_t len) {
@@ -105,6 +108,18 @@
 __global__ void scatter_chars_kernel(const uint32_t *at, const uint8_t *ch, uint64_t n, uint8_t *bases) {
   const uint64_t stride = (uint64_t)gridDim.x * blockDim.x;
   for (uint64_t i = (uint64_t)blockIdx.x * blockDim.x + threadIdx.x; i < n; i += stride) bases[at[i]] = ch[i];
+}
+__global__ void unpack_marked_reads_kernel(const uint8_t *packed, const uint32_t *at, uint64_t n_exc, uint32_t len, uint32_t bytes_per_read,
+                                           uint8_t *bases, uint64_t *off) {
+  const uint64_t stride = (uint64_t)gridDim.x * blockDim.x, total = n_exc * bytes_per_read;
+  for (uint64_t i = (uint64_t)blockIdx.x * blockDim.x + threadIdx.x; i < total; i += stride) {
+    const uint64_t r = at[i / bytes_per_read] / len;
+    const uint32_t kb = (uint32_t)(i % bytes_per_read), k = kb * 4u;
+    const uint32_t b = packed[r * bytes_per_read + kb];
+    uint8_t *o = bases + r * len + k;
+    for (uint32_t q = 0; q < 4u && k + q < len; ++q) o[q] = (uint8_t)((0x54474341u >> (8u * ((b >> (2u * q)) & 3u))) & 0xFFu);
+    if (kb == 0) off[r] = r * (uint64_t)len, off[r + 1] = (r + 1) * (uint64_t)len;
+  }
 }
 
 __global__ void mark_exception_reads_kernel(const uint32_t *at, uint64_t n, uint32_t len, uint32_t *bits) {
@@ -891,6 +906,26 @@
   return pre_mine;
 }
 
+struct QueuedRead {
+  const uint8_t *chars, *codes;
+  uint32_t len;
+  __device__ __forceinline__ uint32_t at(uint32_t j) const {
+    if (codes) return (0x54474341u  >> (8u * ((codes[j >> 2] >> (2u * (j & 3u))) & 3u))) & 0xFFu;
+    return chars[j];
+  }
+};
+__device__ __forceinline__ QueuedRead queued_read(const SeedParams &p, uint32_t read) {
+  QueuedRead r;
+  if (p.packed) {
+    const bool marked = (p.exc_bits[read >> 5] >> (read & 31u)) & 1u;
+    r.chars = p.bases + (uint64_t)read * p.len, r.codes = marked ? nullptr : p.packed + (uint64_t)read * p.bpr, r.len = p.len;
+  } else {
+    const uint64_t off = p.read_off[read];
+    r.chars = p.bases + off, r.codes = nullptr, r.len = (uint32_t)(p.read_off[read + 1] - off);
+  }
+  return r;
+}
+
 __global__ void __launch_bounds__(256) seed_filter_kernel(SeedParams p) {
   extern __shared__ __attribute__((aligned(16))) uint8_t smem[];
   const uint32_t ln = lane_id();
@@ -926,9 +961,8 @@
     const uint32_t read = p.work_queue ? p.work_queue[item] : item;
     if (read == kInvalidRead) continue;
     STAMP_START(prof);
-    const uint64_t off = p.read_off[read];
-    const uint32_t L = (uint32_t)(p.read_off[read + 1] - off);
-    const uint8_t *seq = p.bases + off;
+    const QueuedRead seq = queued_read(p, read);
+    const uint32_t L = seq.len;
     const int S = (int)L - k + 1;
 
     bool shape_ok = S > 0 && R <= S / step;
@@ -961,7 +995,7 @@
           for (int q = 0; q < 4; ++q) {
             uint32_t c = 0, isn = 0;
             if (idx + q < L) {
-              uint32_t code = base_code(seq[idx + q]);
+              uint32_t code = base_code(seq.at(idx + q));
               isn = code >> 2;
               c = code & 3u & (isn - 1u);
               n_fwd_amb += isn & (uint32_t)(idx + q >= (uint32_t)k);
diff --git a/fem_amd/csrc/fem_seed_select.hip.h b/fem_amd/csrc/fem_seed_select.hip.h
--- a/fem_amd/csrc/fem_seed_select.hip.h
+++ b/fem_amd/csrc/fem_seed_select.hip.h
@@ -104,6 +104,18 @@
   return best;
 }
 
+struct PackedArgs {
+  const uint8_t *packed, *bases;
+  const uint32_t *exc_bits;
+  uint32_t bpr, len;
+};
+__device__ __forceinline__ PackedArgs packed_args() {
+  typedef const __attribute__((address_space(4))) SeedParams *ArgPtr;
+  ArgPtr a = (ArgPtr)__builtin_amdgcn_kernarg_segment_ptr();
+  asm volatile("" : "+s"(a));
+  return {a->packed, a->bases, a->exc_bits, a->bpr, a->len};
+}
+
 #ifndef FEM_SELECT_WAVES
 #define FEM_SELECT_WAVES 6
 #endif
@@ -111,7 +123,7 @@
 #define FEM_SELECT_UNROLL 2
 #endif
 
-template <int R, bool BANKED = false>
+template <int R, bool BANKED = false, bool PACKED = false>
 __global__ void __launch_bounds__(256) __attribute__((amdgpu_waves_per_eu(FEM_SELECT_WAVES, 8))) seed_select_kernel(SeedParams p) {
   extern __shared__ __attribute__((aligned(16))) uint8_t smem[];
   const uint32_t ln = lane_id();
@@ -147,24 +159,39 @@
     uint32_t pull = 0;
     if (ln == 0) pull = atomicAdd(p.work_cursor, kReadBlock);
     pull = bcast0(pull);
-    if ((uint64_t)p.read_begin + pull >= p.n_reads) break;
+    if constexpr (PACKED) {
+      if (pull >= p.n_reads - p.read_begin) break;
+    } else {
+      if ((uint64_t)p.read_begin + pull >= p.n_reads) break;
+    }
     const uint32_t r0 = p.read_begin + pull;
     const uint32_t n_blk = p.n_reads - r0 < kReadBlock ? p.n_reads - r0 : kReadBlock;
-    wave_sync_lds();
-    if (ln <= n_blk) boff[ln] = p.read_off[r0 + ln];
-    wave_sync_lds();
+    constexpr bool from_codes = PACKED;
+    if constexpr (!from_codes) {
+      wave_sync_lds();
+      if (ln <= n_blk) boff[ln] = p.read_off[r0 + ln];
+      wave_sync_lds();
+    }
     for (uint32_t sb = 0; sb < n_blk; sb += nb) {
       const uint32_t cnt = n_blk - sb < nb ? n_blk - sb : nb;
       const uint32_t rd0 = r0 + sb;
-      const uint64_t o_first = boff[sb];
-      const uint64_t blk_off = (uint64_t)__builtin_amdgcn_readfirstlane((uint32_t)o_first) |
-                               ((uint64_t)__builtin_amdgcn_readfirstlane((uint32_t)(o_first >> 32)) << 32);
+      uint64_t blk_off = 0;
+      if constexpr (!from_codes) {
+        const uint64_t o_first = boff[sb];
+        blk_off = (uint64_t)__builtin_amdgcn_readfirstlane((uint32_t)o_first) |
+                  ((uint64_t)__builtin_amdgcn_readfirstlane((uint32_t)(o_first >> 32)) << 32);
+      }
       uint32_t my_S = 0, my_flag = 0;
       {
         uint32_t L = 0, base = 0;
         if (ln < cnt) {
-          const uint64_t o0 = boff[sb + ln], o1 = boff[sb + ln + 1u];
-          L = (uint32_t)(o1 - o0), base = (uint32_t)(o0 - blk_off);
+          if constexpr (from_codes) {
+            const PackedArgs pk = packed_args();
+            L = pk.len, base = __umul24(ln, 4u * pk.bpr);
+          } else {
+            const uint64_t o0 = boff[sb + ln], o1 = boff[sb + ln + 1u];
+            L = (uint32_t)(o1 - o0), base = (uint32_t)(o0 - blk_off);
+          }
           const int S = (int)L - kK + 1;
           bool shape_ok = S > 0 && R <= S / kStep;
           if (shape_ok) shape_ok = (S - (kStep - 1)) / kStep - R * kLg + 2 >= 2;
@@ -177,9 +204,39 @@
         }
         if (ln < kReadBlock) r_base[ln] = base, r_len[ln] = L, r_flag[ln] = my_flag, r_pre[ln] = 0;
       }
-      const uint32_t total_chars = (uint32_t)(boff[sb + cnt] - blk_off);
       uint32_t any_n = 0;
-      {
+      if constexpr (from_codes) {
+        const PackedArgs pk = packed_args();
+        const uint8_t *src = pk.packed + (uint64_t)rd0 * pk.bpr;
+        const uint32_t n_words = (cnt * pk.bpr + 3u) >> 2;
+        for (uint32_t q = ln; q < n_words; q += (uint32_t)kWave) {
+          const uint32_t r = __brev(load_u32_unaligned(src + 4u * q));
+          fw[q] = ((r & 0x55555555u) << 1) | ((r >> 1) & 0x55555555u);
+        }
+        uint32_t marked = (pk.exc_bits[rd0 >> 5] >> (rd0 & 31u)) & ((1u << cnt) - 1u);
+        if (marked != 0u) {
+          for (uint32_t q = ln; q < n_words + 2u; q += (uint32_t)kWave) nw[q] = 0;
+          wave_sync_lds();
+          for (; marked; marked &= marked - 1u) {
+            const uint32_t i = (uint32_t)__builtin_ctz(marked);
+            const uint8_t *rs = pk.bases + (uint64_t)(rd0 + i) * pk.len;
+            const uint32_t byte0 = i * pk.bpr;
+            for (uint32_t q = ln; 4u * q < pk.len; q += (uint32_t)kWave) {
+              uint32_t code, nflag;
+              encode4(load_u32_unaligned(rs + 4u * q), code, nflag);
+              const uint32_t left = pk.len - 4u * q;
+              const uint32_t keep = left >= 4u ? 0xFFFFFFFFu : ((1u << (8u * left)) - 1u);
+              nflag &= keep;
+              code &= keep & ~(nflag * 3u);
+              const uint32_t k = byte0 + q, byte_addr = (k >> 2) * 4u + (3u - (k & 3u));
+              ((uint8_t *)fw)[byte_addr] = (uint8_t)pack4(code);
+              ((uint8_t *)nw)[byte_addr] = (uint8_t)pack4(nflag * 3u);
+              any_n |= nflag;
+            }
+          }
+        }
+      } else {
+        const uint32_t total_chars = (uint32_t)(boff[sb + cnt] - blk_off);
         const uint8_t *src = p.bases + blk_off;
         for (uint32_t q = ln; 4u * q < total_chars; q += (uint32_t)kWave) {
           uint32_t code, nflag;
diff --git a/fem_amd/device.py b/fem_amd/device.py
--- a/fem_amd/device.py
+++ b/fem_amd/device.py
@@ -10,7 +10,7 @@
     "fem_dev_open", "fem_dev_close", "fem_strerror", "fem_dev_last_error", "fem_dev_limits",
     "fem_dev_upload_index", "fem_dev_upload_reference", "fem_dev_build_index", "fem_dev_fetch_index",
     "fem_dev_map_batch_submit", "fem_dev_map_batch_wait",
-    "fem_dev_stage_reads", "fem_dev_stage_info", "fem_dev_acquire_stage", "fem_dev_commit_stage", "fem_dev_commit_stage_uniform", "fem_dev_packed_layout", "fem_dev_commit_stage_packed", "fem_dev_map_staged", "fem_dev_sync", "fem_dev_fetch_stats", "fem_dev_fetch", "fem_dev_fetch_packed",
+    "fem_dev_stage_reads", "fem_dev_stage_info", "fem_dev_stage_front", "fem_dev_acquire_stage", "fem_dev_commit_stage", "fem_dev_commit_stage_uniform", "fem_dev_packed_layout", "fem_dev_commit_stage_packed", "fem_dev_map_staged", "fem_dev_sync", "fem_dev_fetch_stats", "fem_dev_fetch", "fem_dev_fetch_packed",
     "fem_dev_fetch_records", "fem_dev_seed_kernel", "fem_dev_index_info",
     "fem_dev_upload_reference_names", "fem_dev_acquire_text_stage", "fem_dev_commit_text_stage", "fem_dev_commit_names_stage", "fem_dev_sam_quals", "fem_dev_reserve_text", "fem_dev_reserve_batch", "fem_set_blocking_waits", "fem_dev_fetch_sam", "fem_dev_fetch_sam_nowait", "fem_dev_sam_wait",
     "fem_dev_set_timing", "fem_dev_reset_timing", "fem_dev_kernel_time", "fem_dev_copy_bandwidth",
@@ -145,6 +145,8 @@
     L.fem_dev_fetch_sam_nowait.argtypes = [vp, C.c_int, C.POINTER(_BatchSam)]
     L.fem_dev_sam_wait.argtypes = [vp, C.c_int]
     L.fem_dev_stage_info.argtypes = [vp, C.c_int, C.POINTER(u64), C.POINTER(C.c_int32)]
+    if hasattr(L, "fem_dev_stage_front"):
+        L.fem_dev_stage_front.argtypes = [vp, C.c_int, C.POINTER(C.c_int32), C.POINTER(C.c_int32)]
     if hasattr(L, "fem_dev_set_pairs"):
         L.fem_dev_set_pairs.argtypes = [vp, C.c_int, C.POINTER(_PairParams)]
         L.fem_dev_fetch_pairs.argtypes = [vp, C.c_int, C.POINTER(_BatchPairs)]
@@ -409,6 +411,11 @@
         self._check(self._L.fem_dev_stage_info(self._h, slot, C.byref(nb), C.byref(pk)))
         return nb.value, bool(pk.value)
 
+    def stage_front(self, slot=0):
+        sp, cr = C.c_int32(0), C.c_int32(0)
+        self._check(self._L.fem_dev_stage_front(self._h, slot, C.byref(sp), C.byref(cr)))
+        return bool(sp.value), bool(cr.value)
+
     def acquire_stage(self, n_reads_cap, n_bases_cap, slot=0):
         pb, po = C.c_void_p(), C.c_void_p()
         self._check(self._L.fem_dev_acquire_stage(self._h, slot, n_reads_cap, n_bases_cap, C.byref(pb), C.byref(po)))
diff --git a/include/fem_hip.h b/include/fem_hip.h
--- a/include/fem_hip.h
+++ b/include/fem_hip.h
@@ -100,6 +100,7 @@
 
 int fem_dev_stage_reads(fem_dev *h, int slot, const fem_read_batch *reads);
 int fem_dev_stage_info(fem_dev *h, int slot, uint64_t *h2d_bytes, int32_t *packed);
+int fem_dev_stage_front(fem_dev *h, int slot, int32_t *select_packed, int32_t *chars_ready);
 int fem_dev_acquire_stage(fem_dev *h, int slot, uint64_t n_reads_cap, uint64_t n_bases_cap, char **bases,
                           uint64_t **offsets);
 int fem_dev_commit_stage(fem_dev *h, int slot, uint64_t n_reads, uint32_t max_len);
```

After: 398.2, median of 6. +1.3%, better.
